# rezashkv/diffusion_pruning

Hardware: AMD Instinct MI355X
Metric: denoise-steps/s (SD-2.1 U-Net forward, 512x512, bs=4 per GPU, 50% channel mask) (higher is better)
Workload: dtype bf16; 1 GPU; BASELINE configs[1]: SD-2.1 UNet2DConditionModelGated.forward, 64x64 latents (512x512), bs=4/GPU, fixed 50% mask (gated semantics), seeded random-init weights, HIP graph replay; global_batch=4, parallelism=replicas x1 (no data-path collective)

## Files before the change

### diffusion_pruning_amd/_lib.py

```python
from __future__ import annotations

import ctypes
import os
from ctypes import POINTER, Structure, c_char_p, c_float, c_int, c_int32, c_int64, c_size_t, c_void_p

_HERE = os.path.dirname(os.path.abspath(__file__))
LIB_PATH = os.environ.get("APTP_LIB") or os.path.join(_HERE, "csrc", "libaptp_hip.so")

ACT_NONE, ACT_SILU, ACT_GEGLU, ACT_GELU = 0, 1, 2, 3
ACT_QUICK_GELU = 5
TILE_AUTO, TILE_128x128, TILE_128x160, TILE_64x128, TILE_64x160, TILE_128x64, TILE_64x64 = range(7)
(TILE_DMA_128x128, TILE_DMA_128x160, TILE_DMA_64x128, TILE_DMA_64x160, TILE_DMA_128x64, TILE_DMA_64x64) = range(7, 13)
(TILE_DMA3_128x128, TILE_DMA3_128x160, TILE_DMA3_64x128, TILE_DMA3_64x160, TILE_DMA3_128x64, TILE_DMA3_64x64) = range(13, 19)
TILE_DMA4_64x128, TILE_DMA4_64x64, TILE_DMA4_128x64 = 24, 25, 26
TILE_HALO_128x160, TILE_HALO_128x128 = 43, 44
(TILE_DMA6_64x64, TILE_DMA8S_64x64, TILE_DMA6_64x128, TILE_DMA6_128x64, TILE_KU2S4_64x64, TILE_KU2S6_64x64, TILE_KU2S4_64x128,
 TILE_KU2S6_64x128, TILE_KU2S4_128x64) = range(45, 54)
TILE_SK_256x160, TILE_SK_256x128 = 64, 65


class ConvGemmParams(Structure):
    _fields_ = [
        ("x", c_void_p), ("ldx", c_int64),
        ("B", c_int32), ("Hin", c_int32), ("Win", c_int32), ("Cin", c_int32),
# ... 26 lines not shown
        ("io_f32", c_int32),
        ("ustat_out", c_void_p), ("ustat_unit", c_int32), ("ustat_units", c_int32), ("ustat_nrep", c_int32),
        ("pad_end", c_int32),
    ]


class GroupNormColStats(Structure):
    _fields_ = [("stats", c_void_p), ("ld", c_int32), ("rows_per_block", c_int32), ("C", c_int32),
                ("ustats", c_void_p), ("unit", c_int32), ("units", c_int32), ("nrep", c_int32)]


class GroupNormParams(Structure):
    _fields_ = [
        ("x", c_void_p), ("ldx", c_int64),
        ("y", c_void_p), ("ldy", c_int64),
        ("B", c_int32), ("HW", c_int32), ("C", c_int32), ("groups", c_int32),
        ("gamma", c_void_p), ("beta", c_void_p),
        ("eps", c_float), ("silu", c_int32),
        ("workspace", c_void_p), ("variant", c_int32),
        ("counters", c_void_p),
        ("colstats", GroupNormColStats * 2),
        ("io_f32", c_int32),
    ]


class LayerNormParams(Structure):
    _fields_ = [
        ("x", c_void_p), ("ldx", c_int64),
        ("y", c_void_p), ("ldy", c_int64),
        ("rows", c_int32), ("C", c_int32),
        ("gamma", c_void_p), ("beta", c_void_p),
        ("eps", c_float),
        ("io_f32", c_int32),
    ]


class AttentionParams(Structure):
    _fields_ = [
        ("q", c_void_p), ("q_stride_b", c_int64), ("q_stride_l", c_int64),
        ("k", c_void_p), ("k_stride_b", c_int64), ("k_stride_l", c_int64),
        ("v", c_void_p), ("v_stride_b", c_int64), ("v_stride_l", c_int64),
        ("o", c_void_p), ("o_stride_b", c_int64), ("o_stride_l", c_int64),
        ("B", c_int32), ("heads", c_int32), ("Lq", c_int32), ("Lk", c_int32),
        ("scale", c_float),
        ("lse", c_void_p),
        ("variant", c_int32),
        ("io_f32", c_int32),
    ]


class GateBwdParams(Structure):
    _fields_ = [
        ("dy", c_void_p), ("lddy", c_int64), ("y0", c_void_p), ("ldy0", c_int64), ("dx", c_void_p), ("lddx", c_int64),
        ("B", c_int32), ("HW", c_int32), ("C", c_int32), ("groups", c_int32),
        ("gate", c_void_p), ("gate_B", c_int32),
        ("dgate_partial", c_void_p),
        ("dgate", c_void_p),
    ]


class GegluParams(Structure):
    _fields_ = [
        ("hg", c_void_p), ("ldhg", c_int64), ("out", c_void_p), ("ldout", c_int64),
        ("dout", c_void_p), ("lddout", c_int64), ("dhg", c_void_p), ("lddhg", c_int64),
        ("B", c_int32), ("HW", c_int32), ("C", c_int32), ("groups", c_int32),
        ("gate", c_void_p), ("gate_B", c_int32),
        ("dgate_partial", c_void_p),
        ("backward", c_int32),
        ("dgate", c_void_p),
    ]


class FfTailParams(Structure):
    _fields_ = [
        ("h", c_void_p), ("ldh", c_int64), ("x", c_void_p), ("ldx", c_int64), ("y", c_void_p), ("ldy", c_int64),
        ("w1", c_void_p), ("b1", c_void_p), ("cs1", c_void_p), ("n1", c_int32), ("ld1", c_int32),
        ("w2", c_void_p), ("b2", c_void_p), ("ld2", c_int32),
        ("w3", c_void_p), ("b3", c_void_p), ("ld3", c_int32),
        ("colstat", c_void_p), ("colstat_ld", c_int32),
        ("M", c_int32), ("C", c_int32),
        ("eps", c_float),
    ]


class WgradParams(Structure):
    _fields_ = [
        ("x", c_void_p), ("ldx", c_int64), ("dy", c_void_p), ("lddy", c_int64), ("dw", c_void_p),
        ("B", c_int32), ("H", c_int32), ("W", c_int32), ("C", c_int32), ("N", c_int32), ("KH", c_int32), ("KW", c_int32),
        ("split_m", c_int32), ("ld_dw", c_int32), ("db", c_void_p), ("slab_stride", c_int64), ("db_stride", c_int64),
        ("stride", c_int32), ("ups", c_int32),
    ]


class FoldRowsParams(Structure):
    _fields_ = [("partials", c_void_p), ("out", c_void_p), ("R", c_int32), ("n_rows", c_int32), ("C", c_int32), ("ld_out", c_int32),
                ("tail_out", c_void_p), ("tail_rows", c_int32), ("pair_split", c_int32), ("tail_n", c_int32)]


class PackDgradParams(Structure):
    _fields_ = [("src", c_void_p), ("dst", c_void_p), ("N", c_int32), ("C", c_int32), ("taps", c_int32), ("src_ld", c_int32),
                ("dst_ld", c_int32), ("dst_rows", c_int32)]


class DepthLerpParams(Structure):
    _fields_ = [
        ("x_in", c_void_p), ("ld_in", c_int64), ("x_out", c_void_p), ("ld_out", c_int64), ("y", c_void_p), ("ld_y", c_int64),
        ("dy", c_void_p), ("ld_dy", c_int64), ("d_in", c_void_p), ("ld_d_in", c_int64), ("d_out", c_void_p), ("ld_d_out", c_int64),
        ("B", c_int32), ("HW", c_int32), ("C", c_int32),
        ("d", c_void_p), ("d_B", c_int32),
        ("dd_partial", c_void_p),
        ("dd", c_void_p),
        ("backward", c_int32),
    ]


class AdamWItem(Structure):
    _fields_ = [("p", c_void_p), ("g", c_void_p), ("m", c_void_p), ("v", c_void_p), ("shadow", c_void_p), ("n", c_int64)]


class AdamWParams(Structure):
    _fields_ = [("items_dev", c_void_p), ("starts_dev", c_void_p), ("n_items", c_int32), ("total_blocks", c_int32),
                ("lr", c_float), ("beta1", c_float), ("beta2", c_float), ("eps", c_float), ("weight_decay", c_float),
                ("step_dev", c_void_p), ("gate_dev", c_void_p), ("grad_scale", c_float)]


class MseParams(Structure):
    _fields_ = [
        ("a", c_void_p), ("lda", c_int64), ("b", c_void_p), ("ldb", c_int64),
        ("rows", c_int64), ("C", c_int32), ("f32", c_int32),
        ("partial", c_void_p), ("out", c_void_p),
        ("g", c_void_p), ("da", c_void_p), ("ldda", c_int64),
        ("backward", c_int32),
    ]


class GroupNormBwdParams(Structure):
    _fields_ = [
        ("x", c_void_p), ("ldx", c_int64), ("dy", c_void_p), ("lddy", c_int64), ("dx", c_void_p), ("lddx", c_int64),
        ("B", c_int32), ("HW", c_int32), ("C", c_int32), ("groups", c_int32),
        ("gamma", c_void_p), ("beta", c_void_p),
        ("eps", c_float), ("silu", c_int32),
        ("fwd_stats", c_void_p),
        ("workspace", c_void_p),
        ("pgrad_partial", c_void_p),
        ("add", c_void_p), ("ldadd", c_int64),
    ]


class UnetPrologueParams(Structure):
    _fields_ = [
        ("sample", c_void_p), ("sample_bf16", c_int32), ("x", c_void_p),
        ("B", c_int32), ("C", c_int32), ("H", c_int32), ("W", c_int32), ("cin_pad", c_int32),
        ("timesteps", c_void_p), ("freqs", c_void_p), ("half", c_int32), ("t_emb", c_void_p),
    ]


class UnetEpilogueParams(Structure):
    _fields_ = [
        ("y", c_void_p), ("ldy", c_int64), ("out", c_void_p), ("out_bf16", c_int32),
        ("B", c_int32), ("C", c_int32), ("H", c_int32), ("W", c_int32),
    ]


class AttentionWideParams(Structure):
    _fields_ = [
        ("q", c_void_p), ("q_stride_b", c_int64), ("q_stride_l", c_int64),
        ("k", c_void_p), ("k_stride_b", c_int64), ("k_stride_l", c_int64),
        ("v", c_void_p), ("v_stride_b", c_int64), ("v_stride_l", c_int64),
        ("o", c_void_p), ("o_stride_b", c_int64), ("o_stride_l", c_int64),
        ("B", c_int32), ("Lq", c_int32), ("Lk", c_int32),
        ("scale", c_float),
        ("io_f32", c_int32),
    ]


class ImageOutParams(Structure):
    _fields_ = [
        ("y", c_void_p), ("ldy", c_int64), ("out", c_void_p), ("out_u8", c_int32),
        ("B", c_int32), ("H", c_int32), ("W", c_int32),
    ]


class ImageInParams(Structure):
    _fields_ = [
        ("x", c_void_p), ("x_bf16", c_int32), ("out", c_void_p), ("out_f32", c_int32),
        ("B", c_int32), ("C", c_int32), ("H", c_int32), ("W", c_int32),
    ]


class LatentDistParams(Structure):
    _fields_ = [
        ("y", c_void_p), ("ldy", c_int64), ("wq", c_void_p), ("bq", c_void_p), ("moments", c_void_p), ("eps", c_void_p),
        ("latents", c_void_p), ("latents_bf16", c_int32), ("scale", c_float),
        ("B", c_int32), ("H", c_int32), ("W", c_int32),
    ]


class AttentionCausalParams(Structure):
    _fields_ = [
        ("q", c_void_p), ("q_stride_b", c_int64), ("q_stride_l", c_int64),
        ("k", c_void_p), ("k_stride_b", c_int64), ("k_stride_l", c_int64),
        ("v", c_void_p), ("v_stride_b", c_int64), ("v_stride_l", c_int64),
        ("o", c_void_p), ("o_stride_b", c_int64), ("o_stride_l", c_int64),
        ("B", c_int32), ("heads", c_int32), ("L", c_int32),
        ("scale", c_float),
        ("io_f32", c_int32),
    ]


class TokenEmbedParams(Structure):
    _fields_ = [
        ("ids", c_void_p), ("tok", c_void_p), ("pos", c_void_p), ("out", c_void_p), ("ldo", c_int64),
        ("B", c_int32), ("L", c_int32), ("C", c_int32), ("vocab", c_int32), ("out_f32", c_int32), ("pos_rows", c_int32),
    ]


class AttentionBiasParams(Structure):
    _fields_ = [
        ("q", c_void_p), ("q_stride_b", c_int64), ("q_stride_l", c_int64),
        ("k", c_void_p), ("k_stride_b", c_int64), ("k_stride_l", c_int64),
        ("v", c_void_p), ("v_stride_b", c_int64), ("v_stride_l", c_int64),
        ("o", c_void_p), ("o_stride_b", c_int64), ("o_stride_l", c_int64),
        ("relbias", c_void_p), ("key_mask", c_void_p),
        ("B", c_int32), ("heads", c_int32), ("L", c_int32),
        ("scale", c_float),
        ("io_f32", c_int32),
    ]


class EmbedLnParams(Structure):
    _fields_ = [
        ("ids", c_void_p), ("word", c_void_p), ("pos", c_void_p), ("gamma", c_void_p), ("beta", c_void_p),
        ("out", c_void_p), ("ldo", c_int64),
        ("B", c_int32), ("L", c_int32), ("C", c_int32), ("vocab", c_int32), ("pos_rows", c_int32), ("pad_id", c_int32),
        ("out_f32", c_int32), ("eps", c_float),
    ]


class MaskedMeanParams(Structure):
    _fields_ = [
        ("x", c_void_p), ("x_stride_b", c_int64), ("x_stride_l", c_int64), ("mask", c_void_p), ("out", c_void_p),
        ("B", c_int32), ("L", c_int32), ("C", c_int32), ("x_f32", c_int32),
    ]


class ColsumParams(Structure):
    _fields_ = [("x", c_void_p), ("ldx", c_int64), ("rows", c_int32), ("C", c_int32), ("partial", c_void_p), ("batch", c_int32)]


class LayerNormPgradParams(Structure):
    _fields_ = [
        ("x", c_void_p), ("ldx", c_int64), ("dy", c_void_p), ("lddy", c_int64),
        ("rows", c_int32), ("C", c_int32), ("eps", c_float), ("partial", c_void_p),
    ]


class LayerNormBwdParams(Structure):
    _fields_ = [
        ("x", c_void_p), ("ldx", c_int64), ("dy", c_void_p), ("lddy", c_int64), ("dx", c_void_p), ("lddx", c_int64),
        ("rows", c_int32), ("C", c_int32),
        ("gamma", c_void_p),
        ("eps", c_float),
        ("add", c_void_p), ("ldadd", c_int64),
    ]


class AttentionBwdParams(Structure):
    _fields_ = [
        ("q", c_void_p), ("q_stride_b", c_int64), ("q_stride_l", c_int64),
        ("k", c_void_p), ("k_stride_b", c_int64), ("k_stride_l", c_int64),
        ("v", c_void_p), ("v_stride_b", c_int64), ("v_stride_l", c_int64),
        ("o", c_void_p), ("o_stride_b", c_int64), ("o_stride_l", c_int64),
        ("dout", c_void_p), ("dout_stride_b", c_int64), ("dout_stride_l", c_int64),
        ("dq", c_void_p), ("dq_stride_b", c_int64), ("dq_stride_l", c_int64),
        ("dk", c_void_p), ("dk_stride_b", c_int64), ("dk_stride_l", c_int64),
        ("dv", c_void_p), ("dv_stride_b", c_int64), ("dv_stride_l", c_int64),
        ("lse", c_void_p), ("delta", c_void_p),
        ("B", c_int32), ("heads", c_int32), ("Lq", c_int32), ("Lk", c_int32),
        ("scale", c_float), ("q_split", c_int32), ("workspace", c_void_p),
    ]


class ImagePatchesParams(Structure):
    _fields_ = [
        ("x", c_void_p), ("nchw", c_int32),
        ("B", c_int32), ("H", c_int32), ("W", c_int32),
        ("S", c_int32), ("P", c_int32),
        ("resize", c_int32),
        ("mean", c_float * 3), ("std", c_float * 3),
        ("out", c_void_p), ("ldo", c_int64),
        ("out_f32", c_int32),
    ]


class VitEmbedLnParams(Structure):
    _fields_ = [
        ("patches", c_void_p), ("ldp", c_int64),
        ("cls", c_void_p), ("pos", c_void_p), ("gamma", c_void_p), ("beta", c_void_p),
        ("out", c_void_p), ("ldo", c_int64),
        ("B", c_int32), ("T", c_int32), ("C", c_int32),
        ("out_f32", c_int32),
        ("eps", c_float),
    ]


class L2NormalizeParams(Structure):
    _fields_ = [("x", c_void_p), ("ldx", c_int64), ("out", c_void_p), ("ldo", c_int64), ("n", c_int32), ("D", c_int32)]


class MmdRbfParams(Structure):
    _fields_ = [
        ("x", c_void_p), ("ldx", c_int64),
        ("y", c_void_p), ("ldy", c_int64),
# ... 10 lines not shown
        ("B", c_int32), ("H", c_int32), ("W", c_int32),
        ("S", c_int32), ("P", c_int32),
        ("xbounds", c_void_p), ("xweights", c_void_p), ("xk", c_int32),
        ("ybounds", c_void_p), ("yweights", c_void_p), ("yk", c_int32),
        ("scratch", c_void_p),
        ("mean", c_float * 3), ("std", c_float * 3),
        ("out", c_void_p), ("ldo", c_int64),
        ("out_f32", c_int32),
    ]


EOS_ARGMAX, EOS_FIRST = 0, 1


class EosPoolLnParams(Structure):
    _fields_ = [
        ("ids", c_void_p),
        ("x", c_void_p), ("x_stride_b", c_int64), ("x_stride_l", c_int64),
        ("gamma", c_void_p), ("beta", c_void_p),
        ("out", c_void_p),
        ("out_act", c_void_p), ("ldo_act", c_int64),
        ("index_out", c_void_p),
        ("B", c_int32), ("L", c_int32), ("C", c_int32),
        ("eos_mode", c_int32), ("eos_token_id", c_int32),
        ("x_f32", c_int32), ("act_f32", c_int32),
        ("eps", c_float),
    ]


class PairedCosineParams(Structure):
    _fields_ = [
        ("a", c_void_p), ("lda", c_int64),
        ("b", c_void_p), ("ldb", c_int64),
        ("cos_out", c_void_p),
        ("sum_out", c_void_p),
        ("n", c_int32), ("D", c_int32),
        ("accumulate", c_int32),
    ]


TRAIN_NO_TABLE = -1


class TrainImageDesc(Structure):
    _fields_ = [
        ("src_off", c_int64),
        ("scratch_off", c_int64),
        ("xtab_off", c_int64), ("ytab_off", c_int64),
        ("H", c_int32), ("W", c_int32),
        ("H1", c_int32), ("W1", c_int32),
        ("top", c_int32), ("left", c_int32), ("flip", c_int32),
        ("xk", c_int32), ("yk", c_int32),
        ("row0", c_int32), ("nrows", c_int32),
        ("reserved", c_int32),
    ]


class TrainImagesParams(Structure):
    _fields_ = [
        ("images", c_void_p), ("images_bytes", c_int64),
        ("desc", c_void_p),
        ("desc_dev", c_void_p),
        ("tables", c_void_p), ("tables_count", c_int64),
        ("scratch", c_void_p), ("scratch_bytes", c_int64),
        ("out", c_void_p),
        ("B", c_int32), ("R", c_int32),
        ("out_f32", c_int32),
    ]


STEP_NOISE_BF16, STEP_NOISE_F32 = 0, 1
STEP_DDIM, STEP_PNDM, STEP_DPMPP = 0, 1, 2
STEP_EPSILON, STEP_V_PREDICTION = 0, 1


class GuidedStepParams(Structure):
    _fields_ = [
        ("noise", c_void_p),
        ("sample", c_void_p),
        ("out", c_void_p),
        ("coef", c_void_p),
        ("slot", c_void_p),
        ("w", c_void_p),
        ("flags", c_void_p),
        ("E", c_void_p),
        ("saved", c_void_p),
        ("n", c_int64),
        ("b", c_int32), ("noise_rows", c_int32),
        ("noise_dtype", c_int32), ("scheduler", c_int32), ("prediction", c_int32), ("do_cfg", c_int32),
        ("guidance_scale", c_float), ("guidance_rescale", c_float),
    ]


PHILOX_F32, PHILOX_BF16, PHILOX_RAW = 0, 1, 2


class PhiloxNormalParams(Structure):
    _fields_ = [
        ("out", c_void_p),
        ("base", c_void_p),
        ("seeds_dev", c_void_p),
        ("draw_dev", c_void_p),
        ("scale_dev", c_void_p),
        ("n", c_int64), ("offset", c_int64), ("draw", c_int64),
        ("b", c_int32), ("out_kind", c_int32),
        ("scale", c_float),
    ]


EXPORTS = [
    ("aptp_conv_gemm", c_int, [POINTER(ConvGemmParams), c_void_p]),
    ("aptp_conv_gemm_workspace_bytes", c_int64, [POINTER(ConvGemmParams)]),
    ("aptp_conv_gemm_suggest_split_k", c_int, [POINTER(ConvGemmParams)]),
    ("aptp_conv_gemm_rowstat_slots", c_int, [POINTER(ConvGemmParams)]),
    ("aptp_conv_gemm_tiles", c_int, [POINTER(ConvGemmParams)]),
    ("aptp_conv_gemm_colstat_rows", c_int, [POINTER(ConvGemmParams)]),
    ("aptp_groupnorm", c_int, [POINTER(GroupNormParams), c_void_p]),
    ("aptp_groupnorm_nchunk", c_int, [c_int]),
    ("aptp_rows_nchunk", c_int, [c_int]),
    ("aptp_groupnorm_workspace_bytes", c_int64, [POINTER(GroupNormParams)]),
    ("aptp_layernorm", c_int, [POINTER(LayerNormParams), c_void_p]),
    ("aptp_attention", c_int, [POINTER(AttentionParams), c_void_p]),
    ("aptp_gate_bwd", c_int, [POINTER(GateBwdParams), c_void_p]),
    ("aptp_geglu", c_int, [POINTER(GegluParams), c_void_p]),
    ("aptp_depth_lerp", c_int, [POINTER(DepthLerpParams), c_void_p]),
    ("aptp_ff_tail_supported", c_int, [c_int, c_int, c_int, c_int, c_int, c_int]),
    ("aptp_ff_tail", c_int, [POINTER(FfTailParams), c_void_p]),
    ("aptp_conv_wgrad_supported", c_int, [POINTER(WgradParams)]),
    ("aptp_conv_wgrad_suggest_split", c_int, [POINTER(WgradParams)]),
    ("aptp_conv_wgrad", c_int, [POINTER(WgradParams), c_void_p]),
    ("aptp_conv_wgrad_many_item_bytes", ctypes.c_int64, []),
    ("aptp_conv_wgrad_many_blocks", c_int, [POINTER(WgradParams)]),
    ("aptp_conv_wgrad_many_fill", c_int, [POINTER(WgradParams), c_void_p, ctypes.c_int32]),
    ("aptp_conv_wgrad_many", c_int, [c_void_p, c_void_p, ctypes.c_int32, ctypes.c_int32, ctypes.c_int32, c_void_p]),
    ("aptp_fold_rows", c_int, [POINTER(FoldRowsParams), c_void_p]),
    ("aptp_pack_dgrad", c_int, [POINTER(PackDgradParams), c_void_p]),
    ("aptp_fold_rows_blocks", c_int, [POINTER(FoldRowsParams)]),
    ("aptp_fold_rows_many", c_int, [c_void_p, c_void_p, c_int32, c_int32, c_void_p]),
    ("aptp_pack_dgrad_blocks", c_int, [POINTER(PackDgradParams)]),
    ("aptp_pack_dgrad_many", c_int, [c_void_p, c_void_p, c_int32, c_int32, c_void_p]),
    ("aptp_adamw_blocks", c_int, [c_int64]),
    ("aptp_adamw_many", c_int, [POINTER(AdamWParams), c_void_p]),
    ("aptp_mse_nblocks", c_int, [c_int64, c_int32]),
    ("aptp_mse", c_int, [POINTER(MseParams), c_void_p]),
    ("aptp_groupnorm_bwd", c_int, [POINTER(GroupNormBwdParams), c_void_p]),
    ("aptp_layernorm_bwd", c_int, [POINTER(LayerNormBwdParams), c_void_p]),
    ("aptp_attention_bwd", c_int, [POINTER(AttentionBwdParams), c_void_p]),
    ("aptp_attention_bwd_q_split", c_int, [POINTER(AttentionBwdParams)]),
    ("aptp_attention_bwd_workspace_bytes", c_size_t, [POINTER(AttentionBwdParams), c_int32]),
    ("aptp_colsum", c_int, [POINTER(ColsumParams), c_void_p]),
    ("aptp_layernorm_pgrad", c_int, [POINTER(LayerNormPgradParams), c_void_p]),
    ("aptp_unet_prologue", c_int, [POINTER(UnetPrologueParams), c_void_p]),
    ("aptp_unet_epilogue", c_int, [POINTER(UnetEpilogueParams), c_void_p]),
    ("aptp_attention_wide", c_int, [POINTER(AttentionWideParams), c_void_p]),
    ("aptp_image_out", c_int, [POINTER(ImageOutParams), c_void_p]),
    ("aptp_image_in", c_int, [POINTER(ImageInParams), c_void_p]),
    ("aptp_latent_dist", c_int, [POINTER(LatentDistParams), c_void_p]),
    ("aptp_attention_causal", c_int, [POINTER(AttentionCausalParams), c_void_p]),
    ("aptp_token_embed", c_int, [POINTER(TokenEmbedParams), c_void_p]),
    ("aptp_attention_bias", c_int, [POINTER(AttentionBiasParams), c_void_p]),
    ("aptp_embed_ln", c_int, [POINTER(EmbedLnParams), c_void_p]),
    ("aptp_masked_mean", c_int, [POINTER(MaskedMeanParams), c_void_p]),
    ("aptp_image_patches", c_int, [POINTER(ImagePatchesParams), c_void_p]),
    ("aptp_vit_embed_ln", c_int, [POINTER(VitEmbedLnParams), c_void_p]),
    ("aptp_l2_normalize", c_int, [POINTER(L2NormalizeParams), c_void_p]),
    ("aptp_mmd_rbf_workspace_bytes", c_int64, [c_int32, c_int32]),
    ("aptp_mmd_rbf", c_int, [POINTER(MmdRbfParams), c_void_p]),
    ("aptp_image_patches_pil_size", c_int, [c_int32, c_int32, c_int32, POINTER(c_int32), POINTER(c_int32), POINTER(c_int32),
                                            POINTER(c_int32)]),
    ("aptp_image_patches_pil", c_int, [POINTER(ImagePatchesPilParams), c_void_p]),
    ("aptp_eos_pool_ln", c_int, [POINTER(EosPoolLnParams), c_void_p]),
    ("aptp_paired_cosine", c_int, [POINTER(PairedCosineParams), c_void_p]),
    ("aptp_train_images", c_int, [POINTER(TrainImagesParams), c_void_p]),
    ("aptp_guided_step", c_int, [POINTER(GuidedStepParams), c_void_p]),
    ("aptp_philox_normal", c_int, [POINTER(PhiloxNormalParams), c_void_p]),
    ("aptp_last_error", c_char_p, []),
    ("aptp_version", c_int, []),
]

_lib = None


class AptpError(RuntimeError):
    pass


def load():
    global _lib
    if _lib is not None:
        return _lib
    import torch
    if not os.path.exists(LIB_PATH):
        raise AptpError(
            f"{LIB_PATH} not found: the HIP extension is the only compute path of diffusion_pruning_amd. "
            "Build it with `make -C diffusion_pruning_amd/csrc` (hipcc, --offload-arch=gfx950).")
    lib = ctypes.CDLL(LIB_PATH)
    for name, res, args in EXPORTS:
        fn = getattr(lib, name)
        fn.restype = res
        fn.argtypes = args
    _lib = lib
    return lib


def check(rc: int, what: str):
    if rc != 0:
        msg = load().aptp_last_error()
        raise AptpError(f"{what} failed (rc={rc}): {msg.decode() if msg else ''}")
```

### diffusion_pruning_amd/csrc/conv_gemm.hip

```cpp
#include "conv_gemm_core.h"

using namespace aptp_cg;

namespace {

template <typename T> struct Elem;
template <> struct Elem<__bf16> { static constexpr int EPC = 8, KS = 64; };
template <> struct Elem<float> { static constexpr int EPC = 4, KS = 32; };

template <int BM, int BN, int WM, int WN, typename T = __bf16>
__global__ __launch_bounds__(256) void conv_gemm_kernel(const KParams p) {
  static_assert(WM * WN == 4, "4 waves per workgroup");
  constexpr int EPC = Elem<T>::EPC, KS = Elem<T>::KS, ES = (int)sizeof(T);
  constexpr bool F32 = sizeof(T) == 4;
  constexpr int WTM = BM / WM, WTN = BN / WN;
  constexpr int MF = WTM / 16, NF = WTN / 16;
  constexpr int A_PASS = BM / 32, B_PASS = BN / 32;
  static_assert(BM % 32 == 0 && BN % 32 == 0 && WTM % 16 == 0 && WTN % 16 == 0, "tile shape");

  __shared__ __attribute__((aligned(16))) T smem[2 * (BM + BN) * KS];
  T* As = smem;
  T* Bs = smem + 2 * BM * KS;

  const int tid = threadIdx.x, lane = tid & 63, wave = tid >> 6;
// ... 957 lines not shown
  k.x2 = (const __bf16*)p->x2; k.ldx2 = p->ldx2; k.Cin2 = p->x2 ? p->Cin2 : 0; k.ncc2 = p->x2 ? p->cin2_pad / ks : 0; k.x2_bytes = 0;
  if (p->x2) {
    APTP_CHECK(p->Cin2 > 0 && p->Cin2 % 8 == 0 && p->cin2_pad % BK == 0 && p->cin2_pad >= p->Cin2 && p->cin2_pad < p->Cin2 + BK,
               "conv_gemm: x2 needs Cin2 (%d) a positive multiple of 8 and cin2_pad (%d) == ceil(Cin2/64)*64", p->Cin2, p->cin2_pad);
    APTP_CHECK(p->ldx2 % 8 == 0 && p->ldx2 >= p->Cin2 && ((uintptr_t)p->x2 % 16) == 0, "conv_gemm: x2 row stride / alignment");
    APTP_CHECK(p->stride == 1 && p->ups == 0 && p->Hout == p->Hin && p->Wout == p->Win,
               "conv_gemm: x2 (second operand read at the output pixel) needs a stride-1, same-size convolution");
    const int64_t x2b = (((int64_t)p->B * p->Hout * p->Wout - 1) * p->ldx2 + p->Cin2) * es;
    APTP_CHECK(x2b < (1ll << 31), "conv_gemm: x2 larger than 2 GiB");
    k.x2_bytes = (int)x2b;
  }
  k.w = (const __bf16*)p->w; k.N = p->N; k.ncc = p->cin_pad / ks; k.nK = p->KH * p->KW * k.ncc + k.ncc2;
  k.Ktot = (int64_t)k.nK * ks;
  k.bias = p->bias; k.rowbias = p->rowbias; k.ld_rowbias = p->ld_rowbias;
  k.colgate = p->colgate; k.gate_group = p->gate_group; k.gate_B = p->gate_B;
  k.act = p->act; k.corr = p->corr; k.corr_B = p->corr_B;
  k.residual = (const __bf16*)p->residual; k.ldres = p->ldres;
  k.depth = p->depth; k.depth_B = p->depth_B; k.depth_in = (const __bf16*)p->depth_in; k.lddin = p->lddin;
  k.y = p->y; k.ldy = p->ldy; k.out_f32 = p->out_f32;
  k.split_k = p->split_k < k.nK ? p->split_k : k.nK;
  k.ws = (float*)p->workspace;
  k.M = (int)M64; k.HW = p->Hout * p->Wout; k.Nout = nout;
  k.ws_ld = p->N;
  APTP_CHECK(p->order >= 0 && p->order <= 3, "conv_gemm: order %d", p->order);
  if (p->order == 0) {
    const int64_t w_bytes = (int64_t)p->N * k.Ktot * 2;
    const int64_t a_bytes = (int64_t)p->B * p->Hin * p->Win * p->Cin * 2;
    k.order = w_bytes > a_bytes ? 1 : 2;
  } else {
    k.order = p->order - 1;
  }
  k.rstat_out = p->rowstat_out; k.rstat_slots = p->rowstat_slots;
  k.ln_stats = p->ln_stats; k.ln_slots = p->ln_slots; k.ln_colsum = p->ln_colsum; k.ln_eps = p->ln_eps;
  k.ln_invC = p->ln_C > 0 ? 1.0f / (float)p->ln_C : 0.f;
  APTP_CHECK(!p->rowstat_out || (!geglu && (!p->out_f32 || f32) && ((uintptr_t)p->rowstat_out % 16) == 0),
             "conv_gemm: rowstat_out needs a bf16, non-GEGLU output and an 8-byte aligned buffer");
  APTP_CHECK(!p->ln_stats || (p->ln_colsum && p->ln_slots > 0 && p->ln_C > 0 && p->KH == 1 && p->KW == 1 &&
                              p->ln_slots % 2 == 0 && ((uintptr_t)p->ln_stats % 16) == 0 && ((uintptr_t)p->ln_colsum % 16) == 0),
             "conv_gemm: folded LayerNorm needs ln_colsum [N], ln_slots > 0, ln_C > 0 and a 1x1 filter");
  k.counters = p->tile_counters;
  k.pf_ptr = ((uintptr_t)p->prefetch & 3) ? nullptr : (const char*)p->prefetch;
  k.pf_bytes = k.pf_ptr ? (p->prefetch_bytes < (1ll << 36) ? p->prefetch_bytes : (1ll << 36)) : 0;
  k.cstat_out = p->colstat_out; k.cstat_ld = p->colstat_ld;
  k.ustat_out = (long long*)p->ustat_out; k.ustat_unit = p->ustat_unit; k.ustat_units = p->ustat_units; k.ustat_nrep = p->ustat_nrep;
  APTP_CHECK(!p->ustat_out || (p->colstat_out && p->ustat_unit > 0 && p->ustat_units * p->ustat_unit >= nout && p->ustat_nrep >= 1 &&
                               (p->ustat_nrep & (p->ustat_nrep - 1)) == 0 && ((uintptr_t)p->ustat_out % 8) == 0),
             "conv_gemm: ustat_out goes with colstat_out; ustat_unit > 0, ustat_units >= ceil(N_out / unit), ustat_nrep a power of two");
  k.epi16 = !p->out_f32 && p->ldy % 8 == 0 && ((uintptr_t)p->y % 16) == 0 && nout % 8 == 0 &&
            (!p->residual || (p->ldres % 8 == 0 && ((uintptr_t)p->residual % 16) == 0)) &&
            (!p->depth || (p->lddin % 8 == 0 && ((uintptr_t)p->depth_in % 16) == 0));
  if (p->epilogue == 1) k.epi16 = 0;
  const int64_t xb = (((int64_t)p->B * p->Hin * p->Win - 1) * p->ldx + p->Cin) * es;
  const int64_t wb = (int64_t)p->N * k.Ktot * es;
  APTP_CHECK(xb < (1ll << 31) && wb < (1ll << 31), "conv_gemm: operand larger than 2 GiB");
  k.x_bytes = (int)xb; k.w_bytes = (int)wb;
  return APTP_OK;
}

template <int BM, int BN>
void launch_tile(const KParams& k, hipStream_t s) {
  const int tiles = ((k.M + BM - 1) / BM) * ((k.N + BN - 1) / BN);
  dim3 grid(tiles * k.split_k, 1, 1);
  if (k.io_f32) hipLaunchKernelGGL((conv_gemm_kernel<BM, BN, 2, 2, float>), grid, dim3(256), 0, s, k);
  else hipLaunchKernelGGL((conv_gemm_kernel<BM, BN, 2, 2>), grid, dim3(256), 0, s, k);
}

template <int BM, int BN, int STAGES>
void launch_tile_dma(const KParams& k, hipStream_t s) {
  const int tiles = ((k.M + BM - 1) / BM) * ((k.N + BN - 1) / BN);
  dim3 grid(tiles * k.split_k, 1, 1);
  hipLaunchKernelGGL((conv_gemm_dma_kernel<BM, BN, 2, 2, STAGES>), grid, dim3(256), 0, s, k);
}

template <int BM, int BN, int WM, int WN, int STAGES = 2>
void launch_tile_dma8(const KParams& k, hipStream_t s) {
  const int tiles = ((k.M + BM - 1) / BM) * ((k.N + BN - 1) / BN);
  dim3 grid(tiles * k.split_k, 1, 1);
  hipLaunchKernelGGL((conv_gemm_dma_kernel<BM, BN, WM, WN, STAGES>), grid, dim3(512), 0, s, k);
}

template <int BM, int BN, int WM, int WN, int STAGES>
void launch_tile_ku2(const KParams& k, hipStream_t s) {
  const int tiles = ((k.M + BM - 1) / BM) * ((k.N + BN - 1) / BN);
  dim3 grid(tiles * k.split_k, 1, 1);
  hipLaunchKernelGGL((conv_gemm_dma_kernel<BM, BN, WM, WN, STAGES, false, 2>), grid, dim3(WM * WN * 64), 0, s, k);
}

template <int BM, int BN, int STAGES>
void launch_tile_ks2(const KParams& k, hipStream_t s) {
  const int tiles = ((k.M + BM - 1) / BM) * ((k.N + BN - 1) / BN);
  dim3 grid(tiles * k.split_k, 1, 1);
  hipLaunchKernelGGL((conv_gemm_dma_kernel<BM, BN, 2, 2, STAGES, false, 1, 2>), grid, dim3(512), 0, s, k);
}

template <int BM, int BN, int WM, int WN, int STAGES>
void launch_tile_pp(const KParams& k, hipStream_t s) {
  const int tiles = ((k.M + BM - 1) / BM) * ((k.N + BN - 1) / BN);
  dim3 grid(tiles * k.split_k, 1, 1);
  hipLaunchKernelGGL((conv_gemm_dma_kernel<BM, BN, WM, WN, STAGES, true>), grid, dim3(512), 0, s, k);
}

}

extern "C" int64_t aptp_conv_gemm_workspace_bytes(const AptpConvGemmParams* p) {
  if (!p || p->split_k <= 1) return 0;
  const int64_t M = (int64_t)p->B * p->Hout * p->Wout;
  const int t = pick_tile(p, (int)M);
  if (is_sk_tile(t))
    return (int64_t)aptp_sk_cus() * 2 * kTiles[t].bm * kTiles[t].bn * (int64_t)sizeof(float);
  int64_t mp = M, np = p->N;
  if (t > 0 && t < kNumTiles) {
    mp = (M + kTiles[t].bm - 1) / kTiles[t].bm * kTiles[t].bm;
    np = ((int64_t)p->N + kTiles[t].bn - 1) / kTiles[t].bn * kTiles[t].bn;
  }
  return (int64_t)p->split_k * mp * np * (int64_t)sizeof(float);
}

extern "C" int aptp_conv_gemm_tiles(const AptpConvGemmParams* p) {
  if (!p) return 0;
  const int64_t M = (int64_t)p->B * p->Hout * p->Wout;
  const int t = pick_tile(p, (int)M);
  if (t <= 0 || t >= kNumTiles) return 0;
  return (int)(((M + kTiles[t].bm - 1) / kTiles[t].bm) * ((p->N + kTiles[t].bn - 1) / kTiles[t].bn));
}

extern "C" int aptp_conv_gemm_colstat_rows(const AptpConvGemmParams* p) {
  if (!p) return 0;
  const int t = pick_tile(p, p->B * p->Hout * p->Wout);
  if (t <= 0 || t >= kNumTiles) return 0;
  return kTiles[t].bm / (kTiles[t].nw / kTiles[t].wn);
}

extern "C" int aptp_conv_gemm_rowstat_slots(const AptpConvGemmParams* p) {
  if (!p) return 0;
  const int t = pick_tile(p, p->B * p->Hout * p->Wout);
  if (t <= 0 || t >= kNumTiles) return 0;
  return ((p->N + kTiles[t].bn - 1) / kTiles[t].bn) * kTiles[t].wn;
}

extern "C" int aptp_conv_gemm_suggest_split_k(const AptpConvGemmParams* p) {
  if (!p) return 1;
  const int M = p->B * p->Hout * p->Wout;
  const int t = pick_tile(p, M);
  const int64_t blocks = (int64_t)((M + kTiles[t].bm - 1) / kTiles[t].bm) * ((p->N + kTiles[t].bn - 1) / kTiles[t].bn);
  const int nK = p->KH * p->KW * (p->cin_pad / BK);
  if (blocks >= 256) return 1;
  int s = (int)((512 + blocks - 1) / blocks);
  const int max_s = nK / 8 > 0 ? nK / 8 : 1;
  if (s > max_s) s = max_s;
  if (s > 32) s = 32;
  return s < 1 ? 1 : s;
}

extern "C" int aptp_conv_gemm(const AptpConvGemmParams* p, aptp_stream_t stream) {
  KParams k;
  const int rc = fill_kparams(p, k);
  if (rc != APTP_OK) return rc;
  if (k.split_k > 1) APTP_CHECK(k.ws != nullptr && ((uintptr_t)k.ws % 16) == 0, "conv_gemm: split_k > 1 needs a 16B-aligned workspace");
  if (k.split_k == 1) k.counters = nullptr;
  k.gn_gamma = p->gn_gamma; k.gn_beta = p->gn_beta; k.gn_groups = p->gn_groups; k.gn_C = p->gn_C; k.gn_silu = p->gn_silu; k.gn_eps = p->gn_eps;
  if (k.gn_gamma) {
    APTP_CHECK(k.gn_beta && k.split_k > 1 && !k.counters && !k.out_f32 && k.act == APTP_ACT_NONE && !k.colgate && !k.corr && !k.residual && !k.depth
               && !k.rstat_out && !k.cstat_out && !k.ln_stats, "conv_gemm: gn_gamma needs a plain bf16 convolution split along K with a reduce launch");
    APTP_CHECK(k.gn_groups > 0 && k.gn_C > 0 && k.gn_C <= k.N && k.gn_C % k.gn_groups == 0 && k.gn_C % 8 == 0 && (k.gn_C / k.gn_groups) % 4 == 0
               && (int64_t)k.HW * (k.gn_C / k.gn_groups) <= 4LL * GN_RED_QPT * GN_RED_NT && k.ldy % 4 == 0,
               "conv_gemm: gn_gamma geometry (C=%d groups=%d HW=%d)", k.gn_C, k.gn_groups, k.HW);
  }
  hipStream_t s = (hipStream_t)stream;
  int t = pick_tile(p, k.M);
  if (t < 0 || t >= kNumTiles) { aptp_set_error("conv_gemm: unknown tile %d", t); return APTP_EINVAL; }
  if (k.io_f32 && t >= APTP_TILE_DMA_128x128) {
    aptp_set_error("conv_gemm: io_f32 (fp32 parity path) runs on the register-staged tiles 1..6 only (got tile %d)", t);
    return APTP_EINVAL;
  }
  if (t >= APTP_TILE_DMA_128x128 && !is_sk_tile(t) && (p->cin_pad * 2 > 8064 || (p->x2 && p->cin2_pad * 2 > 8064))) {
    aptp_set_error("conv_gemm: LDS-DMA tiles need Cin <= 4032 (got cin_pad %d)", p->cin_pad);
    return APTP_EINVAL;
  }
  if (k.rstat_out) {
    const int slots = ((k.N + kTiles[t].bn - 1) / kTiles[t].bn) * kTiles[t].wn;
    if ((k.split_k != 1 && !k.counters) || k.rstat_slots != slots) {
      aptp_set_error("conv_gemm: rowstat_out needs split_k == 1 (or the in-kernel reduction) and rowstat_slots == aptp_conv_gemm_rowstat_slots() (%d), got split_k %d, slots %d",
                     slots, k.split_k, k.rstat_slots);
      return APTP_EINVAL;
    }
  }
  if (k.cstat_out) {
    const int wtm = kTiles[t].bm / (kTiles[t].nw / kTiles[t].wn), wtn = kTiles[t].bn / kTiles[t].wn;
    if (!k.epi16 || k.act == APTP_ACT_GEGLU || (k.split_k != 1 && !k.counters) || k.HW % wtm != 0 || wtn < 32 ||
        k.cstat_ld < k.Nout || ((uintptr_t)k.cstat_out % 8) != 0) {
      aptp_set_error("conv_gemm: colstat_out needs the coalesced bf16 epilogue, no GEGLU, split_k == 1 (or the in-kernel reduction), "
                     "Hout*Wout %% %d == 0 (aptp_conv_gemm_colstat_rows) and colstat_ld >= N", wtm);
      return APTP_EINVAL;
    }
    const int wl = k.act == APTP_ACT_GEGLU ? wtn / 2 : wtn;
    if (k.ustat_out && (wl % k.ustat_unit == 0 ? wl / k.ustat_unit : (wl - 1) / k.ustat_unit + 2) > 64) {
      aptp_set_error("conv_gemm: ustat_unit %d too small for the %d columns of a wave of tile %d (at most 64 units per wave)", k.ustat_unit, wl, t);
      return APTP_EINVAL;
    }
  }
  if (k.act == APTP_ACT_GEGLU && (kTiles[t].bn == 160)) {
    aptp_set_error("conv_gemm: GEGLU cannot use a 160-wide tile");
    return APTP_EINVAL;
  }
  {
    const int tiles_m = (k.M + kTiles[t].bm - 1) / kTiles[t].bm, tiles_n = (k.N + kTiles[t].bn - 1) / kTiles[t].bn;
    APTP_CHECK((int64_t)tiles_m * tiles_n * k.split_k < (1ll << 31) && (int64_t)k.nK * (k.split_k + 1) < (1ll << 31), "conv_gemm: grid too large");
    k.fd_hw = make_fastdiv(k.HW); k.fd_wout = make_fastdiv(k.Wout);
    k.fd_tm = make_fastdiv(tiles_m); k.fd_tn = make_fastdiv(tiles_n); k.fd_sk = make_fastdiv(k.split_k);
    k.fd_perm = make_fastdiv(tiles_n * k.split_k); k.fd_tmn = make_fastdiv(tiles_m * tiles_n);
  }
  static const bool lin_on = !(getenv("APTP_LIN") && getenv("APTP_LIN")[0] == '0');
  if (lin_on && p->epilogue != 2 && p->pad_end == 0 && aptp_lin_eligible(k, t)) {
    const int rc2 = aptp_launch_lin(k, t, s);
    if (rc2 != APTP_OK) return rc2;
    APTP_LAUNCH_CHECK();
    return APTP_OK;
  }
  static const bool lean_on = !(getenv("APTP_CONV_LEAN") && getenv("APTP_CONV_LEAN")[0] == '0');
  if (lean_on && p->epilogue == 0 && p->pad_end == 0 && aptp_conv_lean_eligible(k, t)) {
    const int rc2 = aptp_launch_conv_lean(k, t, s);
    if (rc2 != APTP_OK) return rc2;
  } else
  switch (t) {
    case APTP_TILE_128x128: launch_tile<128, 128>(k, s); break;
    case APTP_TILE_128x160: launch_tile<128, 160>(k, s); break;
    case APTP_TILE_64x128: launch_tile<64, 128>(k, s); break;
    case APTP_TILE_64x160: launch_tile<64, 160>(k, s); break;
    case APTP_TILE_128x64: launch_tile<128, 64>(k, s); break;
    case APTP_TILE_64x64: launch_tile<64, 64>(k, s); break;
    case APTP_TILE_DMA_128x128: launch_tile_dma<128, 128, 2>(k, s); break;
    case APTP_TILE_DMA_128x160: launch_tile_dma<128, 160, 2>(k, s); break;
    case APTP_TILE_DMA_64x128: launch_tile_dma<64, 128, 2>(k, s); break;
    case APTP_TILE_DMA_64x160: launch_tile_dma<64, 160, 2>(k, s); break;
    case APTP_TILE_DMA_128x64: launch_tile_dma<128, 64, 2>(k, s); break;
    case APTP_TILE_DMA_64x64: launch_tile_dma<64, 64, 2>(k, s); break;
    case APTP_TILE_DMA3_128x128: launch_tile_dma<128, 128, 3>(k, s); break;
    case APTP_TILE_DMA3_128x160: launch_tile_dma<128, 160, 3>(k, s); break;
    case APTP_TILE_DMA3_64x128: launch_tile_dma<64, 128, 3>(k, s); break;
    case APTP_TILE_DMA3_64x160: launch_tile_dma<64, 160, 3>(k, s); break;
    case APTP_TILE_DMA3_128x64: launch_tile_dma<128, 64, 3>(k, s); break;
    case APTP_TILE_DMA3_64x64: launch_tile_dma<64, 64, 3>(k, s); break;
    case APTP_TILE_DMA8_128x160: launch_tile_dma8<128, 160, 4, 2>(k, s); break;
    case APTP_TILE_DMA8_256x160: launch_tile_dma8<256, 160, 4, 2>(k, s); break;
    case APTP_TILE_DMA8_128x128: launch_tile_dma8<128, 128, 2, 4>(k, s); break;
    case APTP_TILE_DMA8_256x128: launch_tile_dma8<256, 128, 4, 2>(k, s); break;
    case APTP_TILE_DMA4_64x160: launch_tile_dma<64, 160, 4>(k, s); break;
    case APTP_TILE_DMA4_64x128: launch_tile_dma<64, 128, 4>(k, s); break;
    case APTP_TILE_DMA4_64x64: launch_tile_dma<64, 64, 4>(k, s); break;
    case APTP_TILE_DMA4_128x64: launch_tile_dma<128, 64, 4>(k, s); break;
    case APTP_TILE_DMA4_128x128: launch_tile_dma<128, 128, 4>(k, s); break;
    case APTP_TILE_DMA8R3_128x160: launch_tile_dma8<128, 160, 4, 2, 3>(k, s); break;
    case APTP_TILE_DMA8R4_128x160: launch_tile_dma8<128, 160, 4, 2, 4>(k, s); break;
    case APTP_TILE_DMA8R3_128x128: launch_tile_dma8<128, 128, 2, 4, 3>(k, s); break;
    case APTP_TILE_DMA8R4_128x128: launch_tile_dma8<128, 128, 2, 4, 4>(k, s); break;
    case APTP_TILE_DMA8R3_256x128: launch_tile_dma8<256, 128, 4, 2, 3>(k, s); break;
    case APTP_TILE_PP3_128x160: launch_tile_pp<128, 160, 4, 2, 3>(k, s); break;
    case APTP_TILE_PP4_128x160: launch_tile_pp<128, 160, 4, 2, 4>(k, s); break;
    case APTP_TILE_PP3_128x128: launch_tile_pp<128, 128, 2, 4, 3>(k, s); break;
    case APTP_TILE_PP4_128x128: launch_tile_pp<128, 128, 2, 4, 4>(k, s); break;
    case APTP_TILE_PP4_64x160: launch_tile_pp<64, 160, 4, 2, 4>(k, s); break;
    case APTP_TILE_PP4_64x128: launch_tile_pp<64, 128, 2, 4, 4>(k, s); break;
    case APTP_TILE_PP5_64x160: launch_tile_pp<64, 160, 4, 2, 5>(k, s); break;
    case APTP_TILE_PP4_128x64: launch_tile_pp<128, 64, 4, 2, 4>(k, s); break;
    case APTP_TILE_PP3_256x128: launch_tile_pp<256, 128, 4, 2, 3>(k, s); break;
    case APTP_TILE_PP3_128x256: launch_tile_pp<128, 256, 2, 4, 3>(k, s); break;
    case APTP_TILE_DMA6_64x64: launch_tile_dma<64, 64, 6>(k, s); break;
    case APTP_TILE_DMA8S_64x64: launch_tile_dma<64, 64, 8>(k, s); break;
    case APTP_TILE_DMA6_64x128: launch_tile_dma<64, 128, 6>(k, s); break;
    case APTP_TILE_DMA6_128x64: launch_tile_dma<128, 64, 6>(k, s); break;
    case APTP_TILE_KU2S4_64x64: launch_tile_ku2<64, 64, 2, 2, 4>(k, s); break;
    case APTP_TILE_KU2S6_64x64: launch_tile_ku2<64, 64, 2, 2, 6>(k, s); break;
    case APTP_TILE_KU2S4_64x128: launch_tile_ku2<64, 128, 2, 2, 4>(k, s); break;
    case APTP_TILE_KU2S6_64x128: launch_tile_ku2<64, 128, 2, 2, 6>(k, s); break;
    case APTP_TILE_KU2S4_128x64: launch_tile_ku2<128, 64, 2, 2, 4>(k, s); break;
    case APTP_TILE_KU2S4_128x128: launch_tile_ku2<128, 128, 2, 2, 4>(k, s); break;
    case APTP_TILE_KU2S4_64x160: launch_tile_ku2<64, 160, 2, 2, 4>(k, s); break;
    case APTP_TILE_KU2S4_128x160: launch_tile_ku2<128, 160, 4, 2, 4>(k, s); break;
    case APTP_TILE_KU2S4_128x128W8: launch_tile_ku2<128, 128, 2, 4, 4>(k, s); break;
    case APTP_TILE_KS2S3_64x64: launch_tile_ks2<64, 64, 3>(k, s); break;
    case APTP_TILE_KS2S4_64x64: launch_tile_ks2<64, 64, 4>(k, s); break;
    case APTP_TILE_KS2S3_64x128: launch_tile_ks2<64, 128, 3>(k, s); break;
    case APTP_TILE_KS2S4_64x128: launch_tile_ks2<64, 128, 4>(k, s); break;
    case APTP_TILE_KS2S3_128x64: launch_tile_ks2<128, 64, 3>(k, s); break;
    case APTP_TILE_KS2S3_128x128: launch_tile_ks2<128, 128, 3>(k, s); break;
    case APTP_TILE_SK_256x160: case APTP_TILE_SK_256x128: case APTP_TILE_SK_128x256:
    case APTP_TILE_SKL_256x160: case APTP_TILE_SKL_256x128: case APTP_TILE_SKL_128x256:
    case APTP_TILE_SK_128x160: case APTP_TILE_SKL_128x160: case APTP_TILE_SK_128x128: case APTP_TILE_SKL_128x128: {
      if (k.split_k > 1 && !k.counters) { aptp_set_error("conv_gemm: the stream-K tiles combine in-kernel: split_k > 1 needs tile_counters"); return APTP_EINVAL; }
      const int rc2 = aptp_launch_sk(k, t, s);
      if (rc2 != APTP_OK) return rc2;
      break;
    }
    case APTP_TILE_HALO_128x160:
    case APTP_TILE_HALO_128x128: {
      const int W = p->Wout;
      if (!(p->KH == 3 && p->KW == 3 && p->stride == 1 && p->pad == 1 && p->pad_end == 0 && p->ups == 0 && !p->x2 && W > 0 && 128 % W == 0 &&
            (p->Hout * W) % 128 == 0 && (128 / W + 2) * (W + 2) <= 264)) {
        aptp_set_error("conv_gemm: the halo tiles need a 3x3 / stride-1 / pad-1 convolution without x2 whose width divides 128 (16, 32 or 64)");
        return APTP_EINVAL;
      }
      const int tiles = ((k.M + 127) / 128) * ((k.N + kTiles[t].bn - 1) / kTiles[t].bn);
      if (t == APTP_TILE_HALO_128x160) hipLaunchKernelGGL((conv3x3_halo_kernel<160, 4>), dim3(tiles * k.split_k), dim3(512), 0, s, k);
      else hipLaunchKernelGGL((conv3x3_halo_kernel<128, 4>), dim3(tiles * k.split_k), dim3(512), 0, s, k);
      break;
    }
    default: aptp_set_error("conv_gemm: unknown tile %d", t); return APTP_EINVAL;
  }
  APTP_LAUNCH_CHECK();
  if (k.split_k > 1 && !k.counters) {
    if (k.gn_gamma) {
      hipLaunchKernelGGL(splitk_reduce_gn_kernel, dim3(k.gn_groups, k.B), dim3(GN_RED_NT), 0, s, k);
    } else {
      const int quads = (k.act == APTP_ACT_GEGLU) ? k.N / 8 : k.N / 4;
      const int64_t total = (int64_t)k.M * quads;
      hipLaunchKernelGGL(splitk_reduce_kernel, dim3((unsigned)((total + 255) / 256)), dim3(256), 0, s, k);
    }
    APTP_LAUNCH_CHECK();
  }
  return APTP_OK;
}
```

### diffusion_pruning_amd/csrc/unet_io.hip

```cpp
#include "aptp_common.h"

namespace {

struct IoK {
  const void* sample; int sample_bf16; void* x; int B, C, HW, cpad;
  const float* t; const float* freqs; int half; void* temb;
  int pix_blocks;
};

__global__ __launch_bounds__(256) void unet_prologue_kernel(const IoK p) {
  const int tid = threadIdx.x;
  if ((int)blockIdx.x < p.pix_blocks) {
    const int64_t pix = (int64_t)blockIdx.x * 256 + tid;
    if (pix >= (int64_t)p.B * p.HW) return;
    const int b = (int)(pix / p.HW), r = (int)(pix - (int64_t)b * p.HW);
    __bf16* dst = reinterpret_cast<__bf16*>(p.x) + pix * p.cpad;
    for (int c0 = 0; c0 < p.cpad; c0 += 8) {
      float f[8];
#pragma unroll
      for (int e = 0; e < 8; ++e) {
        const int c = c0 + e;
        float v = 0.f;
        if (c < p.C) {
          const int64_t i = ((int64_t)b * p.C + c) * p.HW + r;
          v = p.sample_bf16 ? (float)reinterpret_cast<const __bf16*>(p.sample)[i] : reinterpret_cast<const float*>(p.sample)[i];
        }
        f[e] = v;
      }
      *reinterpret_cast<uint4*>(dst + c0) = pack_bf16x8(f);
    }
    return;
  }
  const int i = ((int)blockIdx.x - p.pix_blocks) * 256 + tid;
  if (i >= p.B * p.half) return;
  const int b = i / p.half, k = i - b * p.half;
  const float a = p.t[b] * p.freqs[k];
  __bf16* e = reinterpret_cast<__bf16*>(p.temb) + (int64_t)b * 2 * p.half;
  e[k] = (__bf16)cosf(a);
  e[p.half + k] = (__bf16)sinf(a);
}

struct OutK { const float* y; int64_t ld; void* out; int out_bf16; int B, C, HW; };

__global__ __launch_bounds__(256) void unet_epilogue_kernel(const OutK p) {
  const int64_t i = (int64_t)blockIdx.x * 256 + threadIdx.x;
  if (i >= (int64_t)p.B * p.C * p.HW) return;
  const int r = (int)(i % p.HW);
  const int64_t bc = i / p.HW;
  const int c = (int)(bc % p.C), b = (int)(bc / p.C);
  const float v = p.y[((int64_t)b * p.HW + r) * p.ld + c];
  if (p.out_bf16) reinterpret_cast<__bf16*>(p.out)[i] = (__bf16)v;
  else reinterpret_cast<float*>(p.out)[i] = v;
}

struct ImgK { const float* y; int64_t ld; void* out; int out_u8; int B, HW; };

__global__ __launch_bounds__(256) void image_out_kernel(const ImgK p) {
  const int64_t i = (int64_t)blockIdx.x * 256 + threadIdx.x;
  if (i >= (int64_t)p.B * 3 * p.HW) return;
  int64_t pix;
  int c;
  if (p.out_u8) {
    pix = i / 3;
    c = (int)(i - pix * 3);
  } else {
    const int r = (int)(i % p.HW);
    const int64_t bc = i / p.HW;
    c = (int)(bc % 3);
    pix = (bc / 3) * p.HW + r;
  }
  const float y = p.y[pix * p.ld + c];
  const float v = fminf(fmaxf(__fadd_rn(__fmul_rn(y, 0.5f), 0.5f), 0.f), 1.f);
  if (p.out_u8) reinterpret_cast<uint8_t*>(p.out)[i] = (uint8_t)rintf(__fmul_rn(v, 255.f));
  else reinterpret_cast<float*>(p.out)[i] = v;
}

struct ImgInK { const void* x; int x_bf16; void* out; int out_f32; int B, H, W; };

__global__ __launch_bounds__(256) void image_in_kernel(const ImgInK p) {
  const int64_t pix = (int64_t)blockIdx.x * 256 + threadIdx.x;
  const int64_t HW = (int64_t)p.H * p.W;
  if (pix >= (int64_t)p.B * HW) return;
  const int b = (int)(pix / HW), r = (int)(pix - (int64_t)b * HW);
  const int oy = r / p.W, ox = r - oy * p.W;
  float v[32];
#pragma unroll
  for (int e = 27; e < 32; ++e) v[e] = 0.f;
#pragma unroll
  for (int ky = 0; ky < 3; ++ky) {
#pragma unroll
    for (int kx = 0; kx < 3; ++kx) {
      const int iy = oy + ky - 1, ix = ox + kx - 1;
      const bool ok = (unsigned)iy < (unsigned)p.H && (unsigned)ix < (unsigned)p.W;
#pragma unroll
      for (int c = 0; c < 3; ++c) {
        float f = 0.f;
        if (ok) {
          const int64_t i = ((int64_t)b * 3 + c) * HW + (int64_t)iy * p.W + ix;
          f = p.x_bf16 ? (float)reinterpret_cast<const __bf16*>(p.x)[i] : reinterpret_cast<const float*>(p.x)[i];
        }
        v[(ky * 3 + kx) * 3 + c] = f;
      }
    }
  }
  if (p.out_f32) {
    float4* dst = reinterpret_cast<float4*>(reinterpret_cast<float*>(p.out) + pix * 32);
#pragma unroll
    for (int q = 0; q < 8; ++q) dst[q] = make_float4(v[4 * q], v[4 * q + 1], v[4 * q + 2], v[4 * q + 3]);
  } else {
    uint4* dst = reinterpret_cast<uint4*>(reinterpret_cast<__bf16*>(p.out) + pix * 32);
#pragma unroll
    for (int q = 0; q < 4; ++q) dst[q] = pack_bf16x8(v + 8 * q);
  }
}

struct LatK { const float* y; int64_t ld; const float* wq; const float* bq; float* mom; const float* eps; void* lat; int lat_bf16;
              float scale; int B, HW; };

__global__ __launch_bounds__(256) void latent_dist_kernel(const LatK p) {
  const int64_t pix = (int64_t)blockIdx.x * 256 + threadIdx.x;
  if (pix >= (int64_t)p.B * p.HW) return;
  const int b = (int)(pix / p.HW), r = (int)(pix - (int64_t)b * p.HW);
  const float4* src = reinterpret_cast<const float4*>(p.y + pix * p.ld);
  const float4 y0 = src[0], y1 = src[1];
  const float y[8] = {y0.x, y0.y, y0.z, y0.w, y1.x, y1.y, y1.z, y1.w};
  float m[8];
#pragma unroll
  for (int o = 0; o < 8; ++o) {
    float acc = __fmul_rn(p.wq[o * 8], y[0]);
#pragma unroll
    for (int i = 1; i < 8; ++i) acc = __fadd_rn(acc, __fmul_rn(p.wq[o * 8 + i], y[i]));
    m[o] = __fadd_rn(acc, p.bq[o]);
  }
  const int64_t base8 = (int64_t)b * 8 * p.HW + r;
  if (p.mom) {
#pragma unroll
    for (int o = 0; o < 8; ++o) p.mom[base8 + (int64_t)o * p.HW] = m[o];
  }
  if (p.eps) {
    const int64_t base4 = (int64_t)b * 4 * p.HW + r;
#pragma unroll
    for (int c = 0; c < 4; ++c) {
      const float lv = fminf(fmaxf(m[4 + c], -30.f), 20.f);
      const float sd = expf(__fmul_rn(0.5f, lv));
      const float z = __fmul_rn(p.scale, __fadd_rn(m[c], __fmul_rn(sd, p.eps[base4 + (int64_t)c * p.HW])));
      if (p.lat_bf16) reinterpret_cast<__bf16*>(p.lat)[base4 + (int64_t)c * p.HW] = (__bf16)z;
      else reinterpret_cast<float*>(p.lat)[base4 + (int64_t)c * p.HW] = z;
    }
  }
}

struct TokK { const int64_t* ids; const float* tok; const float* pos; void* out; int64_t ldo; int L, C, vocab, out_f32; };

__global__ __launch_bounds__(128) void token_embed_kernel(const TokK p) {
  const int64_t row = blockIdx.x;
  const int l = (int)(row % p.L);
  const int64_t id = p.ids[row];
  const bool ok = id >= 0 && id < p.vocab;
  const float* tr = p.tok + (ok ? id : 0) * (int64_t)p.C;
  const float* pr = p.pos + (int64_t)l * p.C;
  for (int c = 8 * threadIdx.x; c < p.C; c += 8 * 128) {
    float v[8];
    if (ok) {
      const float4 t0 = *reinterpret_cast<const float4*>(tr + c), t1 = *reinterpret_cast<const float4*>(tr + c + 4);
      const float4 q0 = *reinterpret_cast<const float4*>(pr + c), q1 = *reinterpret_cast<const float4*>(pr + c + 4);
      v[0] = __fadd_rn(t0.x, q0.x); v[1] = __fadd_rn(t0.y, q0.y); v[2] = __fadd_rn(t0.z, q0.z); v[3] = __fadd_rn(t0.w, q0.w);
      v[4] = __fadd_rn(t1.x, q1.x); v[5] = __fadd_rn(t1.y, q1.y); v[6] = __fadd_rn(t1.z, q1.z); v[7] = __fadd_rn(t1.w, q1.w);
    } else {
#pragma unroll
      for (int e = 0; e < 8; ++e) v[e] = __builtin_nanf("");
    }
    if (p.out_f32) {
      float4* dst = reinterpret_cast<float4*>(reinterpret_cast<float*>(p.out) + row * p.ldo + c);
      dst[0] = make_float4(v[0], v[1], v[2], v[3]);
      dst[1] = make_float4(v[4], v[5], v[6], v[7]);
    } else {
      *reinterpret_cast<uint4*>(reinterpret_cast<__bf16*>(p.out) + row * p.ldo + c) = pack_bf16x8(v);
    }
  }
}

}

extern "C" int aptp_image_in(const AptpImageInParams* p, aptp_stream_t stream) {
  APTP_CHECK(p && p->x && p->out, "image_in: null pointer");
  APTP_CHECK(p->C == 3, "image_in: pixel_values must have 3 channels (got %d)", p->C);
  APTP_CHECK(p->B > 0 && p->H > 0 && p->W > 0, "image_in: bad extents");
  APTP_CHECK(((uintptr_t)p->x % (p->x_bf16 ? 2 : 4)) == 0 && ((uintptr_t)p->out % 16) == 0, "image_in: pointer alignment");
  const int64_t pix = (int64_t)p->B * p->H * p->W;
  APTP_CHECK((pix + 255) / 256 < (1ll << 31), "image_in: too many pixels");
  ImgInK k;
  k.x = p->x; k.x_bf16 = p->x_bf16 ? 1 : 0; k.out = p->out; k.out_f32 = p->out_f32 ? 1 : 0; k.B = p->B; k.H = p->H; k.W = p->W;
  hipLaunchKernelGGL(image_in_kernel, dim3((unsigned)((pix + 255) / 256)), dim3(256), 0, (hipStream_t)stream, k);
  APTP_LAUNCH_CHECK();
  return APTP_OK;
}

extern "C" int aptp_latent_dist(const AptpLatentDistParams* p, aptp_stream_t stream) {
  APTP_CHECK(p && p->y && p->wq && p->bq, "latent_dist: null pointer");
  APTP_CHECK(p->moments || p->eps, "latent_dist: nothing to write (moments and eps both NULL)");
  APTP_CHECK(!p->eps || p->latents, "latent_dist: eps needs latents");
  APTP_CHECK(p->B > 0 && p->H > 0 && p->W > 0 && p->ldy >= 8 && p->ldy % 4 == 0, "latent_dist: bad extents (ldy >= 8, a multiple of 4)");
  APTP_CHECK(((uintptr_t)p->y % 16) == 0 && ((uintptr_t)p->wq % 4) == 0 && ((uintptr_t)p->bq % 4) == 0 &&
             ((uintptr_t)p->moments % 4) == 0 && ((uintptr_t)p->eps % 4) == 0 && ((uintptr_t)p->latents % (p->latents_bf16 ? 2 : 4)) == 0,
             "latent_dist: pointer alignment");
  APTP_CHECK(p->scale == p->scale, "latent_dist: scale is NaN");
  const int64_t pix = (int64_t)p->B * p->H * p->W;
  APTP_CHECK((int64_t)p->H * p->W < (1ll << 31) && (pix + 255) / 256 < (1ll << 31), "latent_dist: too many pixels");
  LatK k;
  k.y = p->y; k.ld = p->ldy; k.wq = p->wq; k.bq = p->bq; k.mom = p->moments; k.eps = p->eps; k.lat = p->latents;
  k.lat_bf16 = p->latents_bf16 ? 1 : 0; k.scale = p->scale; k.B = p->B; k.HW = p->H * p->W;
  hipLaunchKernelGGL(latent_dist_kernel, dim3((unsigned)((pix + 255) / 256)), dim3(256), 0, (hipStream_t)stream, k);
  APTP_LAUNCH_CHECK();
  return APTP_OK;
}

extern "C" int aptp_image_out(const AptpImageOutParams* p, aptp_stream_t stream) {
  APTP_CHECK(p && p->y && p->out, "image_out: null pointer");
  APTP_CHECK(p->B > 0 && p->H > 0 && p->W > 0 && p->ldy >= 3, "image_out: bad extents (ldy >= 3)");
  APTP_CHECK(((uintptr_t)p->y % 4) == 0 && (p->out_u8 || ((uintptr_t)p->out % 4) == 0), "image_out: pointer alignment");
  APTP_CHECK((int64_t)p->H * p->W < (1ll << 31), "image_out: H * W too large");
  ImgK k;
  k.y = p->y; k.ld = p->ldy; k.out = p->out; k.out_u8 = p->out_u8 ? 1 : 0; k.B = p->B; k.HW = p->H * p->W;
  const int64_t n = (int64_t)k.B * 3 * k.HW;
  APTP_CHECK((n + 255) / 256 < (1ll << 31), "image_out: too many elements");
  hipLaunchKernelGGL(image_out_kernel, dim3((unsigned)((n + 255) / 256)), dim3(256), 0, (hipStream_t)stream, k);
  APTP_LAUNCH_CHECK();
  return APTP_OK;
}

extern "C" int aptp_unet_prologue(const AptpUnetPrologueParams* p, aptp_stream_t stream) {
  APTP_CHECK(p && p->sample && p->x && p->timesteps && p->freqs && p->t_emb, "unet_prologue: null pointer");
  APTP_CHECK(p->B > 0 && p->C > 0 && p->H > 0 && p->W > 0 && p->cin_pad >= p->C && p->cin_pad % 8 == 0 && p->half > 0,
             "unet_prologue: bad extents (cin_pad must be a multiple of 8 and >= C)");
  APTP_CHECK(((uintptr_t)p->x % 16) == 0, "unet_prologue: x alignment");
  IoK k;
  k.sample = p->sample; k.sample_bf16 = p->sample_bf16; k.x = p->x; k.B = p->B; k.C = p->C; k.HW = p->H * p->W; k.cpad = p->cin_pad;
  k.t = p->timesteps; k.freqs = p->freqs; k.half = p->half; k.temb = p->t_emb;
  const int64_t pix = (int64_t)p->B * k.HW;
  k.pix_blocks = (int)((pix + 255) / 256);
  const int tblocks = (p->B * p->half + 255) / 256;
  hipLaunchKernelGGL(unet_prologue_kernel, dim3(k.pix_blocks + tblocks), dim3(256), 0, (hipStream_t)stream, k);
  APTP_LAUNCH_CHECK();
  return APTP_OK;
}

extern "C" int aptp_unet_epilogue(const AptpUnetEpilogueParams* p, aptp_stream_t stream) {
  APTP_CHECK(p && p->y && p->out, "unet_epilogue: null pointer");
  APTP_CHECK(p->B > 0 && p->C > 0 && p->H > 0 && p->W > 0 && p->ldy >= p->C, "unet_epilogue: bad extents");
  OutK k;
  k.y = p->y; k.ld = p->ldy; k.out = p->out; k.out_bf16 = p->out_bf16; k.B = p->B; k.C = p->C; k.HW = p->H * p->W;
  const int64_t n = (int64_t)k.B * k.C * k.HW;
  hipLaunchKernelGGL(unet_epilogue_kernel, dim3((unsigned)((n + 255) / 256)), dim3(256), 0, (hipStream_t)stream, k);
  APTP_LAUNCH_CHECK();
  return APTP_OK;
}

extern "C" int aptp_token_embed(const AptpTokenEmbedParams* p, aptp_stream_t stream) {
  APTP_CHECK(p && p->ids && p->tok && p->pos && p->out, "token_embed: null pointer");
  APTP_CHECK(p->B > 0 && p->L > 0 && p->vocab > 0 && p->C > 0 && p->C % 8 == 0, "token_embed: bad extents (C must be a multiple of 8)");
  APTP_CHECK(p->L <= p->pos_rows, "token_embed: %d tokens but only %d position rows", p->L, p->pos_rows);
  APTP_CHECK(p->ldo >= p->C && p->ldo % 8 == 0, "token_embed: ldo (%lld) must be >= C and a multiple of 8", (long long)p->ldo);
  APTP_CHECK((int64_t)p->B * p->L < (1ll << 31), "token_embed: B * L too large");
  APTP_CHECK(((uintptr_t)p->ids % 8) == 0 && ((uintptr_t)p->tok % 16) == 0 && ((uintptr_t)p->pos % 16) == 0 && ((uintptr_t)p->out % 16) == 0,
             "token_embed: pointer alignment");
  TokK k;
  k.ids = p->ids; k.tok = p->tok; k.pos = p->pos; k.out = p->out; k.ldo = p->ldo;
  k.L = p->L; k.C = p->C; k.vocab = p->vocab; k.out_f32 = p->out_f32;
  hipLaunchKernelGGL(token_embed_kernel, dim3((unsigned)(p->B * p->L)), dim3(128), 0, (hipStream_t)stream, k);
  APTP_LAUNCH_CHECK();
  return APTP_OK;
}
```

### diffusion_pruning_amd/ops.py

```python
from __future__ import annotations

import ctypes
import os
import threading
from dataclasses import dataclass
from typing import Optional

import torch

from . import _lib
from ._lib import ImageInParams, LatentDistParams, UnetEpilogueParams, UnetPrologueParams
from ._lib import ACT_GELU, AttentionCausalParams, TokenEmbedParams
from ._lib import AttentionBiasParams, EmbedLnParams, MaskedMeanParams
from ._lib import ACT_QUICK_GELU, ImagePatchesParams, L2NormalizeParams, MmdRbfParams, VitEmbedLnParams
from ._lib import EOS_ARGMAX, EOS_FIRST, EosPoolLnParams, ImagePatchesPilParams, PairedCosineParams
from ._lib import GuidedStepParams, PhiloxNormalParams
from ._lib import (ACT_GEGLU, ACT_NONE, ACT_SILU, AttentionBwdParams, AttentionParams, ConvGemmParams, DepthLerpParams, GateBwdParams, WgradParams, FfTailParams, FoldRowsParams, PackDgradParams, MseParams,
                   GegluParams, GroupNormBwdParams, GroupNormParams, LayerNormBwdParams, LayerNormParams,
                   ColsumParams, LayerNormPgradParams, AttentionWideParams, ImageOutParams)
from .launch_policy import (BK, SK_AUTO, SK_TILE_FIRST, TUNING, _HALO_TILES, choose_launch, key_of, parse_key,
                            set_entry, set_tuning, splitk_in_kernel, tuning_key, tuning_lookup)

ACT_DTYPE = torch.bfloat16

# ... 94 lines not shown

        def padrows(t):
            if t.shape[0] == n_p:
                return t
            return torch.cat([t, t.new_zeros((n_p - t.shape[0],) + tuple(t.shape[1:]))], 0)
        wh, wg = padrows(wh), padrows(wg)
        w = torch.stack([wh.reshape(n_p // 16, 16, *wh.shape[1:]), wg.reshape(n_p // 16, 16, *wg.shape[1:])], 1)
        w = w.reshape(2 * n_p, *wh.shape[1:])
        if bias is not None:
            bh, bg = padrows(bh), padrows(bg)
            bias = torch.stack([bh.reshape(n_p // 16, 16), bg.reshape(n_p // 16, 16)], 1).reshape(2 * n_p)
    else:
        if out_idx is not None:
            out_idx = out_idx.to(device)
            w = w[out_idx]
            if bias is not None:
                bias = bias[out_idx]
        if in_idx is not None:
            w = w[:, in_idx.to(device)]
        n_live = w.shape[0]
        n_p = round_up(n_live, n_pad_to)
        if n_p != n_live:
            w = torch.cat([w, w.new_zeros((n_p - n_live,) + tuple(w.shape[1:]))], 0)
            if bias is not None:
                bias = torch.cat([bias, bias.new_zeros(n_p - n_live)], 0)
    N, Cin, KH, KW = w.shape
    cin_live = round_up(Cin, cin_pad_to)
    cin_pad = round_up(cin_live, BK)
    packed = torch.zeros(N, KH * KW, cin_pad, dtype=ACT_DTYPE, device=device)
    packed[:, :, :Cin] = w.permute(0, 2, 3, 1).reshape(N, KH * KW, Cin).to(ACT_DTYPE)
    colsum = packed.float().sum(dim=(1, 2)).contiguous() if ln_gamma is not None else None
    return PackedWeight(packed.contiguous(), None if bias is None else bias.contiguous(), N, cin_live, KH, KW, geglu, colsum)


def pack_weight_cat(pw: PackedWeight, w2: torch.Tensor, bias2: Optional[torch.Tensor] = None, *,
                    in_idx: Optional[torch.Tensor] = None) -> PackedWeight:
    assert not pw.geglu and pw.ln_colsum is None and pw.Cin2 == 0
    dev = pw.w.device
    w2 = w2.to(device=dev, dtype=torch.float32).reshape(w2.shape[0], -1)
    if in_idx is not None:
        w2 = w2[:, in_idx.to(dev)]
    n_live, c2 = w2.shape
    assert n_live <= pw.N
    c2_live = round_up(c2, 8)
    c2_pad = round_up(c2_live, BK)
    ext = torch.zeros(pw.N, c2_pad, dtype=ACT_DTYPE, device=dev)
    ext[:n_live, :c2] = w2.to(ACT_DTYPE)
    flat = torch.cat([pw.w.reshape(pw.N, -1), ext], 1).reshape(pw.N, 1, -1).contiguous()
    bias = pw.bias
    if bias2 is not None:
        b2 = torch.zeros(pw.N, dtype=torch.float32, device=dev)
        b2[:n_live] = bias2.to(device=dev, dtype=torch.float32)
        bias = b2 if bias is None else bias + b2
    return PackedWeight(flat, bias, pw.N, pw.Cin, pw.KH, pw.KW, False, None, c2_live, c2_pad, pw.cin_pad)


_ws_cache = {}
_ws_capture_keep = []

LAUNCH_LOG = None
GN_LAUNCH_LOG = None
ATTN_LAUNCH_LOG = None

SPLITK_IN_KERNEL = True
_counters = {}
_N_COUNTERS = 1 << 16


_N_SLABS = int(os.environ.get("APTP_N_SLABS", "16"))
_counters_lock = threading.Lock()


class scratch_domain:

    def __init__(self, name):
        self.name = name

    def __enter__(self):
        self.prev = getattr(_tls, "domain", None)
        _tls.domain = self.name
        return self

    def __exit__(self, *exc):
        _tls.domain = self.prev
        return False


def _domain():
    return getattr(_tls, "domain", None)


def _tile_counters(device):
    key = device.index if device.index is not None else torch.cuda.current_device()
    pool = _counters.get(key)
    if pool is None:
        if torch.cuda.is_current_stream_capturing():
            return None
        with _counters_lock:
            pool = _counters.get(key)
            if pool is None:
                pool = {"buf": torch.zeros(_N_SLABS, _N_COUNTERS, dtype=torch.int32, device=device), "slab": {}}
                _counters[key] = pool
    sid = (torch.cuda.current_stream().cuda_stream, _domain())
    i = pool["slab"].get(sid)
    if i is None:
        with _counters_lock:
            i = pool["slab"].get(sid)
            if i is None:
                if len(pool["slab"]) >= _N_SLABS:
                    return None
                i = pool["slab"][sid] = len(pool["slab"])
    return pool["buf"][i]


GN_DEFAULT_VARIANT = 0
GN_STATS_ONE_LAUNCH = True

ATTN_VARIANT = int(os.environ.get("APTP_ATTN_VARIANT", "0"))

GN_FUSED_FINALIZE = False

EPILOGUE = 0


def _workspace(nbytes: int, device) -> torch.Tensor:
    key = (device.index if device.index is not None else torch.cuda.current_device(), torch.cuda.is_current_stream_capturing(),
           torch.cuda.current_stream().cuda_stream, _domain())
    buf = _ws_cache.get(key)
    if buf is None or buf.numel() < nbytes:
        size = max(nbytes, 1 << 20)
        if key[1] and buf is not None:
            size = max(size, buf.numel() + buf.numel() // 2)
        buf = torch.empty(size, dtype=torch.uint8, device=device)
        if key[1]:
            _ws_capture_keep.append(buf)
        _ws_cache[key] = buf
    return buf


COLSTATS = True
COLSTATS_MIN_HW = 1024


def _root(t: torch.Tensor) -> torch.Tensor:
    return t._base if t._base is not None else t


USTAT = os.environ.get("APTP_USTAT", "1") != "0"
USTAT_NREP = int(os.environ.get("APTP_USTAT_NREP", "8"))
_USTAT_WORDS = 1 << 17
_ustat_arenas = {}


def ustat_begin(device, unit: int):
    if not USTAT or unit <= 0 or torch.device(device).type != "cuda":
        _tls.ustat = None
        return
    capturing = torch.cuda.is_current_stream_capturing()
    key = (torch.device(device).index, torch.cuda.current_stream().cuda_stream, _domain(), capturing)
    ent = _ustat_arenas.get(key)
    if ent is None:
        ent = _ustat_arenas[key] = {"buf": torch.zeros(_USTAT_WORDS, dtype=torch.int64, device=device), "used": 0}
        if capturing:
            _ws_capture_keep.append(ent["buf"])
            ent["used"] = _USTAT_WORDS
    elif ent["used"]:
        ent["buf"][:ent["used"]].zero_()
    _tls.ustat = {"buf": ent["buf"], "off": 0, "unit": int(unit), "ent": ent}


def ustat_end():
    st = getattr(_tls, "ustat", None)
    if st is not None and not st.get("closed"):
        st["closed"] = True
        st["ent"]["used"] = max(st["ent"]["used"], st["off"])


def _ustat_alloc(B: int, nout: int):
    st = getattr(_tls, "ustat", None)
    if st is None or st.get("closed"):
        return None
    unit = st["unit"]
    units = (nout + unit - 1) // unit
    nrep = USTAT_NREP
    while nrep > 1 and nrep * B > 4 * USTAT_NREP:
        nrep //= 2
    n = nrep * B * units * 2
    if st["off"] + n > st["buf"].numel():
        return None
    u = st["buf"][st["off"]:st["off"] + n]
    st["off"] += n
    return u, unit, units, nrep


def _colstats_drop(out: torch.Tensor):
    d = getattr(_root(out), "_aptp_colstats", None)
    if d:
        d.pop(out.storage_offset(), None)


def _colstats_put(out: torch.Tensor, stats: torch.Tensor, rows_per_block: int, ustat=None):
    root = _root(out)
    d = getattr(root, "_aptp_colstats", None)
    if d is None:
        d = {}
        root._aptp_colstats = d
    d[out.storage_offset()] = (stats, rows_per_block, out.shape[3], (out.shape[0], out.shape[1] * out.shape[2]), _ld(out), ustat)


def _colstats_get(x: torch.Tensor, C: int):
    d = getattr(_root(x), "_aptp_colstats", None)
    if not d:
        return None
    segs, off, left, pad = [], x.storage_offset(), x.shape[3], x.shape[3] - C
    while left > 0 and len(segs) < 2:
        rec = d.get(off)
        if rec is None or rec[3] != (x.shape[0], x.shape[1] * x.shape[2]) or rec[4] != _ld(x) or rec[2] > left:
            return None
        segs.append([rec[0], rec[1], rec[2], rec[5] if len(rec) > 5 else None])
        off += rec[2]
        left -= rec[2]
    if left != 0 or segs[-1][2] <= pad:
        return None
    segs[-1][2] -= pad
    return segs


class _PrefetchPlan:

    def __init__(self):
        self.seq = []
        self.i = 0

    def begin(self):
        self.i = 0

    def step(self, w):
        i, self.i = self.i, self.i + 1
        if i < len(self.seq) and self.seq[i] is w:
            nxt = self.seq[i + 1] if i + 1 < len(self.seq) else None
        else:
            del self.seq[i:]
            self.seq.append(w)
            nxt = None
        if nxt is not None and not (PREFETCH_MIN_BYTES <= nxt.numel() * nxt.element_size() <= PREFETCH_MAX_BYTES):
            return None
        return nxt


_tls = threading.local()


def set_prefetch_plan(plan: Optional[_PrefetchPlan]):
    _tls.prefetch_plan = plan
    if plan is not None:
        plan.begin()


def _current_prefetch_plan() -> Optional[_PrefetchPlan]:
    return getattr(_tls, "prefetch_plan", None)


PREFETCH_WEIGHTS = os.environ.get("APTP_PREFETCH", "1") == "1"
PREFETCH_MIN_BYTES = int(os.environ.get("APTP_PREFETCH_MIN", "0"))
PREFETCH_MAX_BYTES = int(os.environ.get("APTP_PREFETCH_MAX", str(12 << 20)))


def conv_gemm(x: torch.Tensor, pw: PackedWeight, *, stride: int = 1, pad: Optional[int] = None, ups: int = 0,
              out: Optional[torch.Tensor] = None, rowbias: Optional[torch.Tensor] = None,
              colgate: Optional[torch.Tensor] = None, gate_group: int = 0, act: int = ACT_NONE,
              corr: Optional[torch.Tensor] = None, residual: Optional[torch.Tensor] = None,
              depth: Optional[torch.Tensor] = None, depth_in: Optional[torch.Tensor] = None,
              out_f32: bool = False, split_k: Optional[int] = None, tile: int = 0, order: int = 0,
              rowstats: bool = False, ln=None, colstats: bool = False, x2: Optional[torch.Tensor] = None,
              prefetch=None, gn=None, pad_end: int = 0):
    if pad_end < 0 or (pad_end and (ups or corr is not None or x2 is not None)):
        raise ValueError("conv_gemm: pad_end must be >= 0 and does not go with ups, corr or x2")
    lib = _lib.load()
    if gn is not None and (colgate is not None or act != ACT_NONE or pw.geglu or corr is not None or residual is not None
                           or depth is not None or out_f32 or rowstats or ln is not None or out is not None):
        raise ValueError("conv_gemm: gn= goes with a plain bf16 convolution (bias / rowbias only)")
    _check_act(x, "conv_gemm x")
    B, Hin, Win, Cx = x.shape
    if Cx != pw.Cin:
        raise ValueError(f"conv_gemm: x has {Cx} channels, packed weight expects {pw.Cin}")
    if pad is None:
        pad = pw.KH // 2
    sh = 1 if ups else 0
    HinE, WinE = Hin << sh, Win << sh
    Hout = (HinE + 2 * pad + pad_end - pw.KH) // stride + 1
    Wout = (WinE + 2 * pad + pad_end - pw.KW) // stride + 1
    if pw.geglu:
        act = ACT_GEGLU
    nout = pw.N // 2 if act == ACT_GEGLU else pw.N
    f32 = x.dtype == torch.float32
    gn_f32 = None
    if f32:
        if pw.w.dtype != torch.float32:
            raise ValueError("conv_gemm: fp32 activations need weights packed under ops.ACT_DTYPE = torch.float32")
        out_f32, colstats, prefetch, gn_f32, gn = True, False, False, gn, None
        if tile not in (0, 1, 2, 3, 4, 5, 6):
            raise ValueError("conv_gemm: the fp32 parity path runs on the register-staged tiles 1..6")
    if out is None:
        out = torch.empty(B, Hout, Wout, nout, dtype=torch.float32 if out_f32 else torch.bfloat16, device=x.device)
    else:
        _colstats_drop(out)
        if tuple(out.shape) != (B, Hout, Wout, nout) or out.stride(3) != 1:
            raise ValueError(f"conv_gemm: out shape {tuple(out.shape)} != {(B, Hout, Wout, nout)}")
        if out.dtype != (torch.float32 if out_f32 else torch.bfloat16):
            raise ValueError("conv_gemm: out dtype mismatch")
    p = ConvGemmParams()
    p.x, p.ldx = x.data_ptr(), _ld(x)
    p.B, p.Hin, p.Win, p.Cin, p.Hout, p.Wout = B, Hin, Win, Cx, Hout, Wout
    p.KH, p.KW, p.stride, p.pad, p.ups = pw.KH, pw.KW, stride, pad, ups
    p.pad_end = pad_end
    p.w, p.N, p.cin_pad = pw.w.data_ptr(), pw.N, pw.cin_pad
    if (x2 is not None) != (pw.Cin2 > 0):
        raise ValueError("conv_gemm: x2 goes with weights packed by pack_weight_cat (and only with them)")
    if x2 is not None:
        _check_act(x2, "conv_gemm x2")
        if tuple(x2.shape) != (B, Hout, Wout, pw.Cin2):
            raise ValueError(f"conv_gemm: x2 shape {tuple(x2.shape)} != {(B, Hout, Wout, pw.Cin2)}")
        p.x2, p.ldx2, p.Cin2, p.cin2_pad = x2.data_ptr(), _ld(x2), pw.Cin2, pw.cin2_pad
    p.bias = None if pw.bias is None else pw.bias.data_ptr()
    if rowbias is not None:
        assert rowbias.dtype == torch.float32 and rowbias.dim() == 2 and rowbias.shape[0] == B and rowbias.stride(1) == 1
        assert rowbias.shape[1] >= pw.N
        p.rowbias, p.ld_rowbias = rowbias.data_ptr(), rowbias.stride(0)
    if colgate is not None:
        assert colgate.dtype == torch.float32 and colgate.dim() == 2 and colgate.is_contiguous()
        assert gate_group > 0 and colgate.shape[1] * gate_group == nout and B % colgate.shape[0] == 0
        p.colgate, p.gate_group, p.gate_B = colgate.data_ptr(), gate_group, colgate.shape[0]
    p.act = act
    if corr is not None:
        assert corr.dtype == torch.float32 and corr.is_contiguous() and corr.shape[1:] == (9, nout)
        assert B % corr.shape[0] == 0
        p.corr, p.corr_B = corr.data_ptr(), corr.shape[0]
    if residual is not None:
        _check_act(residual, "conv_gemm residual")
        assert tuple(residual.shape) == (B, Hout, Wout, nout)
        p.residual, p.ldres = residual.data_ptr(), _ld(residual)
    if depth is not None:
        assert depth.dtype == torch.float32 and depth.dim() == 1 and B % depth.shape[0] == 0 and depth_in is not None
        _check_act(depth_in, "conv_gemm depth_in")
        assert tuple(depth_in.shape) == (B, Hout, Wout, nout)
        p.depth, p.depth_B = depth.data_ptr(), depth.shape[0]
        p.depth_in, p.lddin = depth_in.data_ptr(), _ld(depth_in)
    p.y, p.ldy, p.out_f32 = out.data_ptr(), _ld(out), int(out_f32)
    p.epilogue = EPILOGUE
    p.io_f32 = int(f32)
    if f32:
        for t_, nm in ((x2, "x2"), (residual, "residual"), (depth_in, "depth_in")):
            if t_ is not None and t_.dtype != torch.float32:
                raise ValueError(f"conv_gemm: fp32 parity path: {nm} must be fp32 too")
    if prefetch is False:
        prefetch = None
    elif PREFETCH_WEIGHTS and prefetch is None:
        plan = _current_prefetch_plan()
        if plan is not None:
            prefetch = plan.step(pw.w)
    if prefetch is not None:
        p.prefetch, p.prefetch_bytes = prefetch.data_ptr(), prefetch.numel() * prefetch.element_size()
    plain_linear = pw.KH == 1 and pw.KW == 1 and stride == 1 and not ups and x2 is None and colgate is None and corr is None \
        and rowbias is None and depth is None and not out_f32 and gn is None and (act != ACT_GEGLU or (residual is None and not rowstats))
    p.split_k = 1
    p.tile, sk, in_kernel, p.order = choose_launch(B * Hout * Wout, pw.N, Cx, pw.cin_pad, pw.KH, pw.KW, stride, ups, act, pw.Cin2, pw.cin2_pad,
                                                   plain_linear=plain_linear, f32=f32, tile=tile, split_k=split_k, order=order)
    p.split_k = max(1, int(lib.aptp_conv_gemm_suggest_split_k(ctypes.byref(p)) if sk is None else sk))
    ws = cnt = None
    gn_fused = False
    if gn is not None and FUSE_GN_REDUCE and p.split_k > 1 and Hout * Wout <= GN_REDUCE_MAX_HW:
        gamma, beta, groups, eps_, silu_, Cn = gn
        cgn = Cn // groups
        gn_fused = Cn % 8 == 0 and Cn % groups == 0 and cgn % 4 == 0 and Hout * Wout * cgn <= 4 * 24 * 256 and Cn <= nout
    if gn_fused:
        colstats = False
        p.gn_gamma, p.gn_beta, p.gn_groups, p.gn_C, p.gn_silu, p.gn_eps = gamma.data_ptr(), beta.data_ptr(), groups, Cn, int(silu_), eps_
    want_cols = colstats and COLSTATS and Hout * Wout >= COLSTATS_MIN_HW and act != ACT_GEGLU and not out_f32
    if p.split_k > 1:
        in_kernel = splitk_in_kernel(p.split_k, in_kernel, explicit=split_k is not None, reduce_launch=gn_fused, rowstats=rowstats, colstats=want_cols)
        sk_tile = p.tile >= SK_TILE_FIRST
        if (SPLITK_IN_KERNEL or sk_tile) and (in_kernel or sk_tile) and lib.aptp_conv_gemm_tiles(ctypes.byref(p)) <= _N_COUNTERS:
            cnt = _tile_counters(x.device)
            if cnt is not None:
                p.tile_counters = cnt.data_ptr()
        if sk_tile and cnt is None:
            p.split_k = 1
        else:
            ws = _workspace(lib.aptp_conv_gemm_workspace_bytes(ctypes.byref(p)), x.device)
            p.workspace = ws.data_ptr()
    stats = None
    if rowstats and (p.split_k == 1 or cnt is not None):
        slots = lib.aptp_conv_gemm_rowstat_slots(ctypes.byref(p))
        assert slots % 2 == 0
        stats = torch.empty(slots // 2, B * Hout * Wout, 4, dtype=torch.float32, device=x.device)
        p.rowstat_out, p.rowstat_slots = stats.data_ptr(), slots
    cstats = ustat = None
    if want_cols and (p.split_k == 1 or cnt is not None) and _ld(out) % 8 == 0 and out.data_ptr() % 16 == 0 and nout % 8 == 0 \
            and (residual is None or (_ld(residual) % 8 == 0 and residual.data_ptr() % 16 == 0)) \
            and (depth_in is None or (_ld(depth_in) % 8 == 0 and depth_in.data_ptr() % 16 == 0)) and p.epilogue == 0:
        rpb = lib.aptp_conv_gemm_colstat_rows(ctypes.byref(p))
        if rpb > 0 and (Hout * Wout) % rpb == 0:
            M = B * Hout * Wout
            nblk = (M + rpb - 1) // rpb + 16
            cstats = torch.empty(nblk, nout, 2, dtype=torch.float32, device=x.device)
            p.colstat_out, p.colstat_ld = cstats.data_ptr(), nout
            ustat = _ustat_alloc(B, nout)
            if ustat is not None:
                p.ustat_out, p.ustat_unit, p.ustat_units, p.ustat_nrep = ustat[0].data_ptr(), ustat[1], ustat[2], ustat[3]
    if ln is not None:
        ln_stats, ln_eps = ln
        if pw.ln_colsum is None:
            raise ValueError("conv_gemm: ln= needs weights packed with ln_gamma / ln_beta")
        assert ln_stats.dtype == torch.float32 and ln_stats.is_contiguous() and ln_stats.shape[1] == B * Hout * Wout \
            and ln_stats.shape[2] == 4
        p.ln_stats, p.ln_slots, p.ln_colsum = ln_stats.data_ptr(), 2 * ln_stats.shape[0], pw.ln_colsum.data_ptr()
        p.ln_eps, p.ln_C = ln_eps, Cx
    elif pw.ln_colsum is not None:
        raise ValueError("conv_gemm: weights with a folded LayerNorm need ln=(stats, eps)")
    _lib.check(lib.aptp_conv_gemm(ctypes.byref(p), _stream()), "aptp_conv_gemm")
    if cstats is not None:
        _colstats_put(out, cstats, rpb, ustat)
    if LAUNCH_LOG is not None:
        LAUNCH_LOG.append({"params": p, "flops": 2.0 * B * Hout * Wout * pw.N * (pw.KH * pw.KW * pw.Cin + pw.Cin2),
                           "keep": (x, pw, out, rowbias, colgate, corr, residual, depth, depth_in, ws, stats, ln, cnt, cstats, x2, gn, ustat)})
    if f32 and gn_f32 is not None:
        gn = gn_f32
    if gn is not None and not gn_fused:
        gamma, beta, groups, eps_, silu_, Cn = gn
        return groupnorm(out, gamma, beta, groups, eps_, silu_, C=Cn)
    return (out, stats) if rowstats else out


def linear(x: torch.Tensor, pw: PackedWeight, **kw) -> torch.Tensor:
    B, L, C = x.shape
    out = kw.pop("out", None)
    for k in ("residual", "depth_in"):
        if kw.get(k) is not None:
            kw[k] = kw[k].unsqueeze(2)
    y = conv_gemm(x.unsqueeze(2), pw, pad=0, out=None if out is None else out.unsqueeze(2), **kw)
    if "rowstats" in kw:
        return (y[0].squeeze(2), y[1]) if kw["rowstats"] else (y.squeeze(2), None)
    return y.squeeze(2)


def groupnorm(x: torch.Tensor, gamma: torch.Tensor, beta: torch.Tensor, groups: int, eps: float, silu: bool,
              C: Optional[int] = None, out: Optional[torch.Tensor] = None, keep_stats: bool = False, variant: int = 0):
    lib = _lib.load()
    _check_act(x, "groupnorm x")
    B, H, W, Cp = x.shape
    C = Cp if C is None else C
    assert Cp == round_up(C, 8), f"groupnorm: tensor width {Cp} != roundup8({C})"
    assert gamma.dtype == torch.float32 and beta.dtype == torch.float32 and gamma.numel() == C and beta.numel() == C
    if out is None:
        out = torch.empty(B, H, W, Cp, dtype=x.dtype, device=x.device)
    p = GroupNormParams()
    p.x, p.ldx, p.y, p.ldy = x.data_ptr(), _ld(x), out.data_ptr(), _ld(out)
    p.B, p.HW, p.C, p.groups = B, H * W, C, groups
    p.gamma, p.beta, p.eps, p.silu = gamma.data_ptr(), beta.data_ptr(), eps, int(silu)
    if x.dtype == torch.float32:
        assert out.dtype == torch.float32 and not keep_stats
        p.io_f32, p.variant = 1, 1
        ws = _workspace(lib.aptp_groupnorm_workspace_bytes(ctypes.byref(p)), x.device)
        p.workspace = ws.data_ptr()
        _lib.check(lib.aptp_groupnorm(ctypes.byref(p), _stream()), "aptp_groupnorm(io_f32)")
        return out
    if keep_stats:
        nch = lib.aptp_groupnorm_nchunk(H * W)
        ws_full = torch.empty(B * (nch + 1) * groups * 2, dtype=torch.float32, device=x.device)
        ws = ws_full[:B * nch * groups * 2].view(B, nch, groups, 2)
        p.workspace = ws_full.data_ptr()
        p.variant = 4 if GN_STATS_ONE_LAUNCH else 1
        _lib.check(lib.aptp_groupnorm(ctypes.byref(p), _stream()), "aptp_groupnorm")
        return out, ws
    else:
        ws = _workspace(lib.aptp_groupnorm_workspace_bytes(ctypes.byref(p)), x.device)
    p.variant = variant if variant else GN_DEFAULT_VARIANT
    p.workspace = ws.data_ptr()
    segs = _colstats_get(x, C) if (COLSTATS and variant == 0 and H * W >= COLSTATS_MIN_HW) else None
    if segs is not None:
        for i, (st, rpb, cseg, us) in enumerate(segs):
            p.colstats[i].stats, p.colstats[i].ld, p.colstats[i].rows_per_block, p.colstats[i].C = st.data_ptr(), st.shape[1], rpb, cseg
            if us is not None and us[0].shape[0] == us[3] * B * us[2] * 2:
                p.colstats[i].ustats, p.colstats[i].unit, p.colstats[i].units, p.colstats[i].nrep = us[0].data_ptr(), us[1], us[2], us[3]
        p.variant = 1
    cnt = _tile_counters(x.device) if (GN_FUSED_FINALIZE and B <= _N_COUNTERS) else None
    if cnt is not None:
        p.counters = cnt.data_ptr()
    _lib.check(lib.aptp_groupnorm(ctypes.byref(p), _stream()), "aptp_groupnorm")
    if GN_LAUNCH_LOG is not None:
        GN_LAUNCH_LOG.append({"params": p, "bytes": 2.0 * B * H * W * (C + Cp), "keep": (x, out, gamma, beta, ws, segs, cnt)})
    return (out, ws) if keep_stats else out


def layernorm(x: torch.Tensor, gamma: torch.Tensor, beta: torch.Tensor, eps: float = 1e-5,
              out: Optional[torch.Tensor] = None) -> torch.Tensor:
    lib = _lib.load()
    B, L, C = x.shape
    assert x.dtype in (torch.bfloat16, torch.float32) and x.stride(2) == 1 and x.is_cuda
    ld = x.stride(1) if L > 1 else max(x.stride(1), C)
    assert B == 1 or L == 1 or x.stride(0) == L * ld
    if out is None:
        out = torch.empty(B, L, C, dtype=x.dtype, device=x.device)
    p = LayerNormParams()
    p.io_f32 = int(x.dtype == torch.float32)
    p.x, p.ldx, p.y, p.ldy = x.data_ptr(), ld, out.data_ptr(), out.stride(1) if L > 1 else C
    p.rows, p.C = B * L, C
    p.gamma, p.beta, p.eps = gamma.data_ptr(), beta.data_ptr(), eps
    _lib.check(lib.aptp_layernorm(ctypes.byref(p), _stream()), "aptp_layernorm")
    return out


def attention(q: torch.Tensor, k: torch.Tensor, v: torch.Tensor, heads: int, scale: Optional[float] = None,
              out: Optional[torch.Tensor] = None, lse: Optional[torch.Tensor] = None) -> torch.Tensor:
    lib = _lib.load()
    B, Lq = q.shape[0], q.shape[1]
    Lk = k.shape[1]
    for t in (q, k, v):
        assert t.dtype == q.dtype and t.dtype in (torch.bfloat16, torch.float32) and t.stride(2) == 1 and t.shape[2] == heads * 64 and t.is_cuda
    if out is None:
        out = torch.empty(B, Lq, heads * 64, dtype=q.dtype, device=q.device)
    p = AttentionParams()
    p.io_f32 = int(q.dtype == torch.float32)
    _set_views(p, q=q, k=k, v=v, o=out)
    p.B, p.heads, p.Lq, p.Lk = B, heads, Lq, Lk
    p.scale = (1.0 / 8.0) if scale is None else scale
    p.variant = ATTN_VARIANT
    if lse is not None:
        assert lse.dtype == torch.float32 and lse.is_contiguous() and tuple(lse.shape) == (B, heads, Lq)
        p.lse = lse.data_ptr()
    if ATTN_LAUNCH_LOG is not None and not p.io_f32:
        ATTN_LAUNCH_LOG.append({"params": p, "flops": 4.0 * B * heads * Lq * Lk * 64, "keep": (q, k, v, out, lse), "Lk": Lk})
    _lib.check(lib.aptp_attention(ctypes.byref(p), _stream()), "aptp_attention")
    return out


FUSE_GN_REDUCE = os.environ.get("APTP_FUSE_GN_REDUCE", "0") != "0"
GN_REDUCE_MAX_HW = 256


FUSE_TAIL = os.environ.get("APTP_FUSE_TAIL", "0") != "0"
FUSE_TAIL_MIN_ROWS = int(os.environ.get("APTP_FUSE_TAIL_MIN_ROWS", "16384"))


def ff_tail_supported(h: torch.Tensor, pw1: PackedWeight, pw2: PackedWeight, pw3: PackedWeight) -> bool:
    if not (FUSE_TAIL and h.is_cuda and h.dtype == torch.bfloat16 and pw1.geglu and pw1.ln_colsum is not None):
        return False
    B, L, C = h.shape
    if B * L < FUSE_TAIL_MIN_ROWS or pw2.N != C or pw3.N != C or pw2.bias is None or pw3.bias is None or pw1.bias is None:
        return False
    return bool(_lib.load().aptp_ff_tail_supported(B * L, C, pw1.N, pw1.cin_pad, pw2.cin_pad, pw3.cin_pad))


def ff_tail(h: torch.Tensor, x: torch.Tensor, pw1: PackedWeight, pw2: PackedWeight, pw3: PackedWeight, eps: float = 1e-5,
            out: Optional[torch.Tensor] = None, colstats: bool = False) -> torch.Tensor:
    lib = _lib.load()
    B, L, C = h.shape
    for t, nm in ((h, "h"), (x, "x")):
        assert t.dtype == torch.bfloat16 and t.is_cuda and tuple(t.shape) == (B, L, C) and t.stride(2) == 1, nm
    if out is None:
        out = torch.empty(B, L, C, dtype=torch.bfloat16, device=h.device)
    else:
        _colstats_drop(out.unsqueeze(2))
    assert tuple(out.shape) == (B, L, C) and out.dtype == torch.bfloat16 and out.stride(2) == 1
    p = FfTailParams()
    for name, t in (("h", h), ("x", x), ("y", out)):
        _, _, _, ld = _rows(t)
        assert B == 1 or t.stride(0) == L * ld, "rows must be uniformly strided"
        setattr(p, name, t.data_ptr())
        setattr(p, "ld" + name, ld)
    p.w1, p.b1, p.cs1, p.n1, p.ld1 = pw1.w.data_ptr(), pw1.bias.data_ptr(), pw1.ln_colsum.data_ptr(), pw1.N, pw1.cin_pad
    p.w2, p.b2, p.ld2 = pw2.w.data_ptr(), pw2.bias.data_ptr(), pw2.cin_pad
    p.w3, p.b3, p.ld3 = pw3.w.data_ptr(), pw3.bias.data_ptr(), pw3.cin_pad
    p.M, p.C, p.eps = B * L, C, eps
    cstats = None
    if colstats and COLSTATS and L >= COLSTATS_MIN_HW and L % 64 == 0:
        cstats = torch.empty(B * L // 64, C, 2, dtype=torch.float32, device=h.device)
        p.colstat, p.colstat_ld = cstats.data_ptr(), C
    _lib.check(lib.aptp_ff_tail(ctypes.byref(p), _stream()), "aptp_ff_tail")
    if cstats is not None:
        _colstats_put(out.unsqueeze(2), cstats, 64)
    if LAUNCH_LOG is not None:
        LAUNCH_LOG.append({"params": p, "fn": "aptp_ff_tail", "flops": 2.0 * B * L * (C * pw1.N + pw2.Cin * C + C * C),
                           "keep": (h, x, out, pw1, pw2, pw3, cstats)})
    return out


def unet_prologue(sample: torch.Tensor, timesteps: torch.Tensor, freqs: torch.Tensor, cin_pad: int):
    lib = _lib.load()
    assert sample.is_cuda and sample.dim() == 4 and sample.dtype in (torch.float32, torch.bfloat16)
    sample = sample.contiguous()
    B, C, H, W = sample.shape
    t = timesteps.to(device=sample.device, dtype=torch.float32).contiguous()
    assert t.numel() == B and freqs.dtype == torch.float32 and freqs.is_contiguous()
    x = torch.empty(B, H, W, cin_pad, dtype=torch.bfloat16, device=sample.device)
    temb = torch.empty(B, 2 * freqs.numel(), dtype=torch.bfloat16, device=sample.device)
    p = UnetPrologueParams()
    p.sample, p.sample_bf16, p.x = sample.data_ptr(), int(sample.dtype == torch.bfloat16), x.data_ptr()
    p.B, p.C, p.H, p.W, p.cin_pad = B, C, H, W, cin_pad
    p.timesteps, p.freqs, p.half, p.t_emb = t.data_ptr(), freqs.data_ptr(), freqs.numel(), temb.data_ptr()
    _lib.check(lib.aptp_unet_prologue(ctypes.byref(p), _stream()), "aptp_unet_prologue")
    return x, temb


def unet_epilogue(y: torch.Tensor, channels: int, out_dtype: torch.dtype, out: Optional[torch.Tensor] = None) -> torch.Tensor:
    lib = _lib.load()
    assert y.is_cuda and y.dtype == torch.float32 and y.dim() == 4 and y.is_contiguous() and out_dtype in (torch.float32, torch.bfloat16)
    B, H, W, ld = y.shape
    if out is None:
        out = torch.empty(B, channels, H, W, dtype=out_dtype, device=y.device)
    assert tuple(out.shape) == (B, channels, H, W) and out.dtype == out_dtype and out.is_contiguous() and out.is_cuda
    p = UnetEpilogueParams()
    p.y, p.ldy, p.out, p.out_bf16 = y.data_ptr(), ld, out.data_ptr(), int(out_dtype == torch.bfloat16)
    p.B, p.C, p.H, p.W = B, channels, H, W
    _lib.check(lib.aptp_unet_epilogue(ctypes.byref(p), _stream()), "aptp_unet_epilogue")
    return out


WIDE_HEAD = 512
ATTN_WIDE_LAUNCH_LOG = None


def attention_wide(q: torch.Tensor, k: torch.Tensor, v: torch.Tensor, scale: Optional[float] = None,
                   out: Optional[torch.Tensor] = None) -> torch.Tensor:
    lib = _lib.load()
    B, Lq = q.shape[0], q.shape[1]
    Lk = k.shape[1]
    for t, nm in ((q, "q"), (k, "k"), (v, "v")):
        if t.dim() != 3 or t.dtype != q.dtype or t.dtype not in (torch.bfloat16, torch.float32) or t.stride(2) != 1 \
                or t.shape[2] != WIDE_HEAD or t.shape[0] != B or not t.is_cuda:
            raise ValueError(f"attention_wide: {nm} must be a CUDA bf16 (or fp32) [B, L, 512] view with contiguous channels, "
                             f"got {t.dtype} {tuple(t.shape)} strides {t.stride()}")
    if v.shape[1] != Lk:
        raise ValueError("attention_wide: k and v must have the same length")
    if out is None:
        out = torch.empty(B, Lq, WIDE_HEAD, dtype=q.dtype, device=q.device)
    if tuple(out.shape) != (B, Lq, WIDE_HEAD) or out.dtype != q.dtype or out.stride(2) != 1:
        raise ValueError("attention_wide: out must be [B, Lq, 512] of q's dtype with contiguous channels")
    p = AttentionWideParams()
    p.io_f32 = int(q.dtype == torch.float32)
    _set_views(p, q=q, k=k, v=v, o=out)
    p.B, p.Lq, p.Lk = B, Lq, Lk
    p.scale = WIDE_HEAD ** -0.5 if scale is None else float(scale)
    if ATTN_WIDE_LAUNCH_LOG is not None and not p.io_f32:
        ATTN_WIDE_LAUNCH_LOG.append({"params": p, "flops": 4.0 * B * Lq * Lk * WIDE_HEAD, "keep": (q, k, v, out)})
    _lib.check(lib.aptp_attention_wide(ctypes.byref(p), _stream()), "aptp_attention_wide")
    return out


def image_out(y: torch.Tensor, out_dtype: torch.dtype = torch.float32, out: Optional[torch.Tensor] = None) -> torch.Tensor:
    lib = _lib.load()
    if not (y.is_cuda and y.dtype == torch.float32 and y.dim() == 4 and y.shape[3] >= 3 and y.stride(3) == 1
            and y.is_contiguous()):
        raise ValueError(f"image_out: expected a contiguous CUDA fp32 [B, H, W, >=3] tensor, got {y.dtype} {tuple(y.shape)}")
    if out_dtype not in (torch.float32, torch.uint8):
        raise ValueError("image_out: out_dtype is torch.float32 or torch.uint8")
    B, H, W, ld = y.shape
    shape = (B, H, W, 3) if out_dtype == torch.uint8 else (B, 3, H, W)
    if out is None:
        out = torch.empty(shape, dtype=out_dtype, device=y.device)
    if tuple(out.shape) != shape or out.dtype != out_dtype or not out.is_contiguous():
        raise ValueError(f"image_out: out must be a contiguous {out_dtype} {shape} tensor")
    p = ImageOutParams()
    p.y, p.ldy, p.out, p.out_u8 = y.data_ptr(), ld, out.data_ptr(), int(out_dtype == torch.uint8)
    p.B, p.H, p.W = B, H, W
    _lib.check(lib.aptp_image_out(ctypes.byref(p), _stream()), "aptp_image_out")
    return out


def image_in(x: torch.Tensor, out_f32: bool = False, out: Optional[torch.Tensor] = None) -> torch.Tensor:
    lib = _lib.load()
    if not (x.is_cuda and x.dim() == 4 and x.dtype in (torch.float32, torch.bfloat16) and x.is_contiguous()):
        raise ValueError(f"image_in: expected a contiguous CUDA fp32 / bf16 NCHW tensor, got {x.dtype} {tuple(x.shape)}")
    B, C, H, W = x.shape
    dt = torch.float32 if out_f32 else torch.bfloat16
    if out is None:
        out = torch.empty(B, H, W, 32, dtype=dt, device=x.device)
    if tuple(out.shape) != (B, H, W, 32) or out.dtype != dt or not out.is_contiguous():
        raise ValueError(f"image_in: out must be a contiguous {dt} {(B, H, W, 32)} tensor")
    p = ImageInParams()
    p.x, p.x_bf16, p.out, p.out_f32 = x.data_ptr(), int(x.dtype == torch.bfloat16), out.data_ptr(), int(out_f32)
    p.B, p.C, p.H, p.W = B, C, H, W
    _lib.check(lib.aptp_image_in(ctypes.byref(p), _stream()), "aptp_image_in")
    return out


def pack_conv_in_im2col(w: torch.Tensor, bias: Optional[torch.Tensor], device=None) -> PackedWeight:
    O, C, KH, KW = w.shape
    if (C, KH, KW) != (3, 3, 3):
        raise ValueError(f"pack_conv_in_im2col: expected a [O, 3, 3, 3] weight, got {tuple(w.shape)}")
    w2 = torch.zeros(O, 32, dtype=torch.float32, device=w.device)
    w2[:, :27] = w.detach().float().permute(0, 2, 3, 1).reshape(O, 27)
    return pack_weight(w2, None if bias is None else bias.detach(), device=device)


def latent_dist(y: torch.Tensor, wq: torch.Tensor, bq: torch.Tensor, eps: Optional[torch.Tensor] = None,
                scale: float = 1.0, moments: bool = True, latents_dtype: torch.dtype = torch.float32,
                moments_out: Optional[torch.Tensor] = None, latents_out: Optional[torch.Tensor] = None):
    lib = _lib.load()
    if not (y.is_cuda and y.dtype == torch.float32 and y.dim() == 4 and y.shape[3] >= 8 and y.is_contiguous()):
        raise ValueError(f"latent_dist: expected a contiguous CUDA fp32 [B, h, w, >=8] tensor, got {y.dtype} {tuple(y.shape)}")
    B, H, W, ld = y.shape
    wq = wq.to(device=y.device, dtype=torch.float32).reshape(8, 8).contiguous()
    bq = bq.to(device=y.device, dtype=torch.float32).reshape(8).contiguous()
    p = LatentDistParams()
    p.y, p.ldy, p.wq, p.bq = y.data_ptr(), ld, wq.data_ptr(), bq.data_ptr()
    p.B, p.H, p.W, p.scale = B, H, W, float(scale)
    mom = lat = None
    if moments:
        mom = moments_out if moments_out is not None else torch.empty(B, 8, H, W, dtype=torch.float32, device=y.device)
        if tuple(mom.shape) != (B, 8, H, W) or mom.dtype != torch.float32 or not mom.is_contiguous():
            raise ValueError(f"latent_dist: moments must be a contiguous fp32 {(B, 8, H, W)} tensor")
        p.moments = mom.data_ptr()
    if eps is not None:
        if tuple(eps.shape) != (B, 4, H, W) or eps.dtype != torch.float32 or not eps.is_contiguous() or eps.device != y.device:
            raise ValueError(f"latent_dist: eps must be a contiguous fp32 {(B, 4, H, W)} tensor on {y.device}")
        if latents_dtype not in (torch.float32, torch.bfloat16):
            raise ValueError("latent_dist: latents_dtype is torch.float32 or torch.bfloat16")
        lat = latents_out if latents_out is not None else torch.empty(B, 4, H, W, dtype=latents_dtype, device=y.device)
        if tuple(lat.shape) != (B, 4, H, W) or lat.dtype != latents_dtype or not lat.is_contiguous():
            raise ValueError(f"latent_dist: latents must be a contiguous {latents_dtype} {(B, 4, H, W)} tensor")
        p.eps, p.latents, p.latents_bf16 = eps.data_ptr(), lat.data_ptr(), int(latents_dtype == torch.bfloat16)
    _lib.check(lib.aptp_latent_dist(ctypes.byref(p), _stream()), "aptp_latent_dist")
    return mom, lat


CAUSAL_MAX_L = 128


def attention_causal(q: torch.Tensor, k: torch.Tensor, v: torch.Tensor, heads: int, scale: Optional[float] = None,
                     out: Optional[torch.Tensor] = None) -> torch.Tensor:
    lib = _lib.load()
    B, L = q.shape[0], q.shape[1]
    if out is None:
        out = torch.empty(B, L, heads * 64, dtype=q.dtype, device=q.device)
    _check_heads64_views(q, k, v, out, B, L, heads, "attention_causal")
    p = AttentionCausalParams()
    p.io_f32 = int(q.dtype == torch.float32)
    _set_views(p, q=q, k=k, v=v, o=out)
    p.B, p.heads, p.L = B, heads, L
    p.scale = 0.125 if scale is None else scale
    _lib.check(lib.aptp_attention_causal(ctypes.byref(p), _stream()), "aptp_attention_causal")
    return out


def token_embed(ids: torch.Tensor, tok: torch.Tensor, pos: torch.Tensor, out_f32: bool = False,
                out: Optional[torch.Tensor] = None) -> torch.Tensor:
    lib = _lib.load()
    if ids.dtype != torch.int64 or ids.dim() != 2 or not ids.is_contiguous() or not ids.is_cuda:
        raise ValueError(f"token_embed: ids must be a contiguous CUDA int64 [B, L] tensor, got {ids.dtype} {tuple(ids.shape)}")
    B, L = ids.shape
    V, C = tok.shape
    for t, nm in ((tok, "tok"), (pos, "pos")):
        if t.dtype != torch.float32 or t.dim() != 2 or not t.is_contiguous() or t.shape[1] != C or t.device != ids.device:
            raise ValueError(f"token_embed: {nm} must be a contiguous fp32 [rows, {C}] tensor on the ids' device")
    if pos.shape[0] < L:
        raise ValueError(f"token_embed: {L} tokens but only {pos.shape[0]} positions")
    odt = torch.float32 if out_f32 else torch.bfloat16
    if out is None:
        out = torch.empty(B, L, C, dtype=odt, device=ids.device)
    elif tuple(out.shape) != (B, L, C) or out.dtype != odt or not out.is_contiguous():
        raise ValueError(f"token_embed: out must be a contiguous {odt} [{B}, {L}, {C}] tensor")
    p = TokenEmbedParams()
    p.ids, p.tok, p.pos, p.out, p.ldo = ids.data_ptr(), tok.data_ptr(), pos.data_ptr(), out.data_ptr(), C
    p.B, p.L, p.C, p.vocab, p.out_f32, p.pos_rows = B, L, C, V, int(out_f32), pos.shape[0]
    _lib.check(lib.aptp_token_embed(ctypes.byref(p), _stream()), "aptp_token_embed")
    return out


BIAS_MAX_L = 512


def _check_heads64_views(q, k, v, out, B: int, L: int, heads: int, name: str):
    for t in (q, k, v, out):
        if t.dtype != q.dtype or t.dtype not in (torch.bfloat16, torch.float32) or t.dim() != 3 or t.stride(2) != 1 \
                or tuple(t.shape) != (B, L, heads * 64) or not t.is_cuda or t.device != q.device:
            raise ValueError(f"{name}: q, k, v and out must be {q.dtype} [B, L, {heads * 64}] views with contiguous "
                             f"channels on {q.device}, got {t.dtype} {tuple(t.shape)} strides {t.stride()} on {t.device}")


def _check_mask(mask: Optional[torch.Tensor], B: int, L: int, device, name: str):
    if mask is not None and (mask.dtype != torch.float32 or tuple(mask.shape) != (B, L) or not mask.is_contiguous()
                             or mask.device != device):
        raise ValueError(f"{name}: the mask must be a contiguous fp32 [{B}, {L}] tensor on {device}, got {mask.dtype} "
                         f"{tuple(mask.shape)} on {mask.device}")


def attention_bias(q: torch.Tensor, k: torch.Tensor, v: torch.Tensor, heads: int, relbias: torch.Tensor,
                   key_mask: Optional[torch.Tensor] = None, scale: Optional[float] = None,
                   out: Optional[torch.Tensor] = None) -> torch.Tensor:
    lib = _lib.load()
    B, L = q.shape[0], q.shape[1]
    if out is None:
        out = torch.empty(B, L, heads * 64, dtype=q.dtype, device=q.device)
    _check_heads64_views(q, k, v, out, B, L, heads, "attention_bias")
    if relbias.dtype != torch.float32 or tuple(relbias.shape) != (heads, 2 * L - 1) or not relbias.is_contiguous() \
            or relbias.device != q.device:
        raise ValueError(f"attention_bias: relbias must be a contiguous fp32 [{heads}, {2 * L - 1}] tensor on {q.device}, got "
                         f"{relbias.dtype} {tuple(relbias.shape)} on {relbias.device}")
    _check_mask(key_mask, B, L, q.device, "attention_bias")
    p = AttentionBiasParams()
    p.io_f32 = int(q.dtype == torch.float32)
    _set_views(p, q=q, k=k, v=v, o=out)
    p.relbias, p.key_mask = relbias.data_ptr(), (None if key_mask is None else key_mask.data_ptr())
    p.B, p.heads, p.L = B, heads, L
    p.scale = 0.125 if scale is None else scale
    _lib.check(lib.aptp_attention_bias(ctypes.byref(p), _stream()), "aptp_attention_bias")
    return out


def embed_ln(ids: torch.Tensor, word: torch.Tensor, pos: torch.Tensor, gamma: torch.Tensor, beta: torch.Tensor,
             eps: float = 1e-5, pad_id: int = 1, out_f32: bool = False, out: Optional[torch.Tensor] = None) -> torch.Tensor:
    lib = _lib.load()
    if ids.dtype != torch.int64 or ids.dim() != 2 or not ids.is_contiguous() or not ids.is_cuda:
        raise ValueError(f"embed_ln: ids must be a contiguous CUDA int64 [B, L] tensor, got {ids.dtype} {tuple(ids.shape)}")
    B, L = ids.shape
    V, C = word.shape
    for t, nm, shp in ((word, "word", (V, C)), (pos, "pos", (pos.shape[0], C)), (gamma, "gamma", (C,)), (beta, "beta", (C,))):
        if t.dtype != torch.float32 or tuple(t.shape) != shp or not t.is_contiguous() or t.device != ids.device:
            raise ValueError(f"embed_ln: {nm} must be a contiguous fp32 {shp} tensor on the ids' device")
    if pos.shape[0] <= L + pad_id:
        raise ValueError(f"embed_ln: {L} tokens with pad id {pad_id} need {L + pad_id + 1} positions, have {pos.shape[0]}")
    odt = torch.float32 if out_f32 else torch.bfloat16
    if out is None:
        out = torch.empty(B, L, C, dtype=odt, device=ids.device)
    elif tuple(out.shape) != (B, L, C) or out.dtype != odt or not out.is_contiguous():
        raise ValueError(f"embed_ln: out must be a contiguous {odt} [{B}, {L}, {C}] tensor")
    p = EmbedLnParams()
    p.ids, p.word, p.pos, p.gamma, p.beta = ids.data_ptr(), word.data_ptr(), pos.data_ptr(), gamma.data_ptr(), beta.data_ptr()
    p.out, p.ldo = out.data_ptr(), C
    p.B, p.L, p.C, p.vocab, p.pos_rows, p.pad_id, p.out_f32, p.eps = B, L, C, V, pos.shape[0], pad_id, int(out_f32), eps
    _lib.check(lib.aptp_embed_ln(ctypes.byref(p), _stream()), "aptp_embed_ln")
    return out


def masked_mean(x: torch.Tensor, mask: Optional[torch.Tensor] = None, out: Optional[torch.Tensor] = None) -> torch.Tensor:
    lib = _lib.load()
    if x.dtype not in (torch.bfloat16, torch.float32) or x.dim() != 3 or x.stride(2) != 1 or not x.is_cuda:
        raise ValueError(f"masked_mean: x must be a CUDA bf16 or fp32 [B, L, C] tensor with contiguous channels, got {x.dtype} "
                         f"{tuple(x.shape)}")
    B, L, C = x.shape
    _check_mask(mask, B, L, x.device, "masked_mean")
    if out is None:
        out = torch.empty(B, C, dtype=torch.float32, device=x.device)
    elif tuple(out.shape) != (B, C) or out.dtype != torch.float32 or not out.is_contiguous() or out.device != x.device:
# ... 1176 lines not shown
```

### diffusion_pruning_amd/unet.py

```python
from __future__ import annotations

import os

import math
from dataclasses import dataclass, field
from typing import Any, Dict, List, Optional, Tuple, Union

import torch
import torch.nn as nn

from . import ops
from .gates import DepthGate, LinearWidthGate, WidthGate
from .modules import LinearP, PlannedModule, _capturing, _Params, _PlanCache, _versions
from .ops import PackedWeight



class Conv2dP(_Params):
    def __init__(self, cin, cout, k):
        super().__init__()
        self.in_channels, self.out_channels, self.kernel_size = cin, cout, (k, k)
        self.weight = nn.Parameter(torch.empty(cout, cin, k, k))
        self.bias = nn.Parameter(torch.empty(cout))

# ... 1118 lines not shown
    def from_config(cls, config: Optional[dict] = None, **kwargs):
        cfg = dict(config or {})
        cfg.update(kwargs)
        return cls(**cfg)

    @torch.no_grad()
    def init_synthetic(self, seed: int = 0, w_std: float = 0.02, beta_std: float = 0.1):
        g = torch.Generator().manual_seed(seed)
        for name, prm in self.named_parameters():
            owner = self.get_submodule(name.rsplit(".", 1)[0])
            if isinstance(owner, NormP):
                if name.endswith(".weight"):
                    prm.fill_(1.0)
                else:
                    prm.copy_(torch.randn(prm.shape, generator=g) * beta_std)
            elif name.endswith(".weight"):
                prm.copy_(torch.randn(prm.shape, generator=g) * w_std)
            else:
                prm.copy_(torch.randn(prm.shape, generator=g) * (0.5 * w_std))
        self.invalidate_plans()
        return self

    def invalidate_plans(self):
        self._misc.clear()
        self._batched.clear()
        for m in self.modules():
            if m is not self and hasattr(m, "invalidate"):
                m.invalidate()

    def _apply(self, fn, *a, **k):
        out = super()._apply(fn, *a, **k)
        self.invalidate_plans()
        return out

    def load_state_dict(self, *a, **k):
        out = super().load_state_dict(*a, **k)
        self.invalidate_plans()
        return out

    def state_dict(self, *a, **k):
        pk = self.__dict__.get("_pk")
        if pk is not None:
            pk.export_()
        return super().state_dict(*a, **k)

    def save_pretrained(self, save_directory: str, **unused):
        from . import checkpoint
        root, sub = os.path.split(os.path.normpath(save_directory))
        checkpoint.save_pretrained(self, root, subfolder=sub)

    @classmethod
    def from_pretrained(cls, pretrained_model_name_or_path: str, subfolder: Optional[str] = None, **kwargs):
        from . import checkpoint
        return checkpoint.from_pretrained(pretrained_model_name_or_path, subfolder=subfolder, cls=cls, **kwargs)

    def freeze(self):
        for name, param in self.named_parameters():
            if "gate_f" not in name:
                param.requires_grad = False

    def _containers(self):
        return list(self.down_blocks) + [self.mid_block] + list(self.up_blocks)

    def get_structure(self):
        if len(self.structure["width"]) == 0:
            structure = {"width": [], "depth": []}
            for m in self._containers():
                s = m.get_gate_structure()
                assert len(s) == 2 and len(s["width"]) == len(s["depth"])
                structure["width"] = structure["width"] + s["width"]
                structure["depth"] = structure["depth"] + s["depth"]
            self.structure = structure
        return self.structure

    def set_structure(self, arch_vectors, prefetch_hosts: bool = True):
        width_vectors, depth_vectors = arch_vectors["width"], arch_vectors["depth"]
        self._installed_structure = {"width": list(width_vectors), "depth": list(depth_vectors)}
        self._structure_epoch = self.__dict__.get("_structure_epoch", 0) + 1
        self._host_map = {}
        if prefetch_hosts:
            self._prefetch_hosts(width_vectors, depth_vectors)
        for m in self._containers():
            s = m.get_gate_structure()
            block_vectors = {"width": [], "depth": []}
            for i in range(len(s["width"])):
                for j in range(len(s["width"][i])):
                    assert s["width"][i][j] == width_vectors[0].shape[1]
                    block_vectors["width"].append(width_vectors.pop(0))
            for i in range(len(s["depth"])):
                if s["depth"][i] == [1]:
                    block_vectors["depth"].append(depth_vectors.pop(0))
            m.set_gate_structure(block_vectors)
        self._attach_hosts()

    def _prefetch_hosts(self, width_vectors, depth_vectors):
        self._host_map = {}
        tensors = list(width_vectors) + list(depth_vectors)
        if not tensors:
            return
        if all(t.device.type == "cpu" for t in tensors):
            return
        flat = torch.cat([t.detach().float().reshape(-1) for t in tensors]).cpu()
        off = 0
        for t in tensors:
            n = t.numel()
            self._host_map[id(t)] = flat[off:off + n].reshape(t.shape)
            off += n

    def _attach_hosts(self):
        hm = getattr(self, "_host_map", None)
        if not hm:
            return
        for m in self.modules():
            if isinstance(m, (WidthGate, DepthGate)):
                h = hm.get(id(m.gate_f))
                if h is not None:
                    m.set_host_value(h)
        self._host_map = {}

    def count_macs(self, latent_h: int, latent_w: Optional[int] = None, text_len: int = 77):
        from . import macs
        macs.assign_module_macs(self, latent_h, latent_w, text_len)
        sanity = self.calc_macs()
        self.prunable_macs_list = [[e / sanity["prunable_macs"] for e in elem] for elem in self.get_prunable_macs()]
        self.resource_info_dict = sanity
        return sanity

    def calc_macs(self):
        from . import macs
        return macs.unet_calc_macs(self)

    def get_prunable_macs(self):
        from . import macs
        return macs.unet_get_prunable_macs(self)

    def get_block_utilization(self):
        from . import macs
        return macs.unet_get_block_utilization(self)

    def _resnets(self):
        return [m for m in self.modules() if isinstance(m, ResnetBlock2DWidthGated)]

    def _transformers(self):
        return [m for m in self.modules() if isinstance(m, Transformer2DModelWidthGated)]

    def _misc_packs(self, dev):
        ver = () if self.__dict__.get("_pk") is not None else \
            tuple(p._version for mod in (self.conv_in, self.time_embedding, self.conv_norm_out, self.conv_out) for p in mod.parameters())
        m = self._misc.get(str(dev), ver)
        if m is None:
            cin_pad = ops.round_up(self.in_channels, 8)
            m = {"cin_pad": cin_pad}
            m["conv_in"] = ops.pack_weight(self.conv_in.weight.detach(), self.conv_in.bias.detach(), device=dev)
            te = self.time_embedding
            m["t1"] = ops.pack_weight(te.linear_1.weight.detach(), te.linear_1.bias.detach(), device=dev)
            m["t2"] = ops.pack_weight(te.linear_2.weight.detach(), te.linear_2.bias.detach(), device=dev)
            m["gn_g"], m["gn_b"] = _f32(self.conv_norm_out.weight).to(dev), _f32(self.conv_norm_out.bias).to(dev)
            m["conv_out"] = ops.pack_weight(self.conv_out.weight.detach(), self.conv_out.bias.detach(), device=dev)
            half = self.conv_in.out_channels // 2
            m["freqs"] = torch.exp(-math.log(10000.0) * torch.arange(half, dtype=torch.float32, device=dev) / half)
            self._misc.put(str(dev), ver, m)
        return m

    def _batched_packs(self, dev):
        resnets, trans = self._resnets(), self._transformers()
        for r in resnets:
            r.semantics = self.semantics
        rplans = [r.plan(dev) for r in resnets if not (r.depth_gated and (r.dropped or r._depth_state()[0] == 0.0))]
        live_res = [r for r in resnets if not (r.depth_gated and (r.dropped or r._depth_state()[0] == 0.0))]
        live_tr = [t for t in trans if not (t.depth_gated and (t.dropped or t._depth_state()[0] == 0.0))]
        tplans = [t.plan(dev) for t in live_tr]
        key = (tuple(id(p) for p in rplans), tuple(id(p) for p in tplans), str(dev))
        bp = self._batched.get(key, ())
        if bp is not None:
            return bp
        bp = {"key": key, "plans": (rplans, tplans)}
        ws, bs, slots, off = [], [], [], 0
        for r, pl in zip(live_res, rplans):
            npad = pl["c_pad"]
            w, b = pl["temb_w"], pl["temb_b"]
            if w.shape[0] != npad:
                w = torch.cat([w, w.new_zeros(npad - w.shape[0], w.shape[1])], 0)
                b = torch.cat([b, b.new_zeros(npad - b.shape[0])], 0)
            ws.append(w); bs.append(b)
            slots.append((id(r), off, npad))
            off += npad
        bp["temb_pw"] = ops.pack_weight(torch.cat(ws, 0), torch.cat(bs, 0), device=dev)
        bp["temb_slots"] = slots
        ws, slots, off, gates = [], [], 0, []
        for t, pl in zip(live_tr, tplans):
            w = pl["a2_kv_w"]
            ws.append(w)
            slots.append((id(t.transformer_blocks[0].attn2), off, w.shape[0]))
            off += w.shape[0]
            gates.append((t.transformer_blocks[0].attn2.gate, pl["a2_dense_gate"], pl["a2_heads"]))
        if ws:
            bp["kv_pw"] = ops.pack_weight(torch.cat(ws, 0), None, device=dev)
        bp["kv_slots"] = slots
        bp["kv_gates"] = gates
        return self._batched.put(key, (), bp)

    def _project_context(self, encoder_hidden_states, bp, dev) -> CtxBundle:
        ehs = encoder_hidden_states.to(device=dev, dtype=ops.ACT_DTYPE).contiguous()
        reusable = not any(dense for (_, dense, _) in bp["kv_gates"])
        ctx = CtxBundle(ehs=ehs, key=bp["key"] if reusable else None)
        if bp["kv_slots"]:
            gkw = {}
            if any(dense for (_, dense, _) in bp["kv_gates"]):
                cols = []
                for gate, dense, hl in bp["kv_gates"]:
                    g = gate.gate_f.detach().to(device=dev, dtype=torch.float32) if dense else None
                    bg = max(gt.gate_f.shape[0] for gt, d_, _ in bp["kv_gates"] if d_)
                    if g is None:
                        g = torch.ones(bg, hl, device=dev)
                    elif g.shape[0] != bg:
                        g = g.repeat(bg // g.shape[0], 1)
                    cols.append(g.repeat(1, 2))
                gkw = dict(colgate=torch.cat(cols, 1).contiguous(), gate_group=64)
            kv_all = ops.linear(ehs, bp["kv_pw"], **gkw)
            for aid, off, n in bp["kv_slots"]:
                ctx.kv[aid] = kv_all[..., off:off + n]
        return ctx

    @torch.no_grad()
    def precompute_context(self, encoder_hidden_states: torch.Tensor) -> CtxBundle:
        dev = encoder_hidden_states.device
        return self._project_context(encoder_hidden_states, self._batched_packs(dev), dev)

    def _register_cat_slots(self, B, H, W, c_in, dev):
        if _ft_mode(self):
            return None
        skips = [None]
        for blk in self.down_blocks:
            for i in range(len(blk.resnets)):
                skips.append(blk.attentions[i] if blk.has_cross_attention else blk.resnets[i])
            if blk.downsamplers is not None:
                skips.append(blk.downsamplers[0])
        prev = self.mid_block.resnets[-1]
        conv_in_slot = None
        for blk in self.up_blocks:
            for i, resnet in enumerate(blk.resnets):
                cs = resnet.skip_connection_dim
                slot = _CatSlot(resnet.in_channels - cs, cs)
                prev.__dict__["_out_dst"] = (slot, 0)
                sk = skips.pop()
                if sk is None:
                    conv_in_slot = slot
                else:
                    sk.__dict__["_out_dst"] = (slot, 1)
                prev = blk.attentions[i] if blk.has_cross_attention else resnet
            if blk.upsamplers is not None:
                prev = blk.upsamplers[0]
        return None if conv_in_slot is None else conv_in_slot.view(1, B, H, W, c_in, dev)

    def _forward_ft(self, sample, timestep, encoder_hidden_states, return_dict):
        from . import autograd as AG
        dev = sample.device
        B = sample.shape[0]
        misc = self._misc_packs(dev)
        for r in self._resnets():
            r.semantics = self.semantics

        def bwd(name, param):
            def get():
                if name not in misc:
                    misc[name] = ops.pack_weight_dgrad(param.detach(), device=dev)
                return misc[name]
            return get
        timesteps = timestep
        if not torch.is_tensor(timesteps):
            timesteps = torch.tensor([timesteps], dtype=torch.int64, device=dev)
        elif timesteps.dim() == 0:
            timesteps = timesteps[None].to(dev)
        timesteps = timesteps.to(dev).expand(B)
        ang = timesteps.float()[:, None] * misc["freqs"][None, :]
        t_emb = torch.cat([torch.cos(ang), torch.sin(ang)], dim=-1).to(torch.bfloat16)
        te = self.time_embedding
        e1 = _cw(self, t_emb[None], te.linear_1.weight, te.linear_1.bias, misc["t1"], bwd("t1_bwd", te.linear_1.weight), pad=0, out_f32=True)
        e1 = torch.nn.functional.silu(e1).to(torch.bfloat16)
        e2 = _cw(self, e1, te.linear_2.weight, te.linear_2.bias, misc["t2"], bwd("t2_bwd", te.linear_2.weight), pad=0, out_f32=True)
        temb = TembBundle(emb_silu=torch.nn.functional.silu(e2)[0].to(torch.bfloat16))
        ctx = CtxBundle(ehs=encoder_hidden_states.to(device=dev, dtype=torch.bfloat16).contiguous())
        x = torch.zeros(B, sample.shape[2], sample.shape[3], misc["cin_pad"], dtype=torch.bfloat16, device=dev)
        x[..., :self.in_channels] = sample.permute(0, 2, 3, 1)
        live_in = torch.arange(self.in_channels, device=dev)
        h = _nchw(_cw(self, x, self.conv_in.weight, self.conv_in.bias, misc["conv_in"], bwd("conv_in_bwd", self.conv_in.weight),
                            live_in=live_in))
        res_samples = (h,)
        for blk in self.down_blocks:
            h, res = blk(hidden_states=h, temb=temb, encoder_hidden_states=ctx)
            res_samples += res
        h = self.mid_block(h, temb, encoder_hidden_states=ctx)
        for blk in self.up_blocks:
            n_res = len(blk.resnets)
            res = res_samples[-n_res:]
            res_samples = res_samples[:-n_res]
            h = blk(hidden_states=h, temb=temb, res_hidden_states_tuple=res, encoder_hidden_states=ctx)
        a = _gnw(self, _nhwc(h), self.conv_norm_out.weight, self.conv_norm_out.bias, misc["gn_g"], misc["gn_b"],
                                  self.conv_norm_out.num_groups, self.conv_norm_out.eps, True, self.conv_norm_out.num_channels, None)
        live_out = torch.arange(self.out_channels, device=dev)
        y = _cw(self, a, self.conv_out.weight, self.conv_out.bias, misc["conv_out"], bwd("conv_out_bwd", self.conv_out.weight),
                      out_f32=True, live_out=live_out)
        out = y[..., :self.out_channels].permute(0, 3, 1, 2).to(sample.dtype)
        if not return_dict:
            return (out,)
        return UNet2DConditionOutput(sample=out)

    def forward(self, sample: torch.Tensor, timestep, encoder_hidden_states: torch.Tensor, class_labels=None,
                timestep_cond=None, attention_mask=None, cross_attention_kwargs=None, added_cond_kwargs=None,
                down_block_additional_residuals=None, mid_block_additional_residual=None, encoder_attention_mask=None,
                return_dict: bool = True):
        if attention_mask is not None or encoder_attention_mask is not None or class_labels is not None \
                or down_block_additional_residuals is not None or mid_block_additional_residual is not None:
            raise NotImplementedError("only the arguments the APTP trainer/pipeline pass are supported")
        dev = sample.device
        B = sample.shape[0]
        plans = self.__dict__.setdefault("_pf_plans", {})
        mode = torch.is_grad_enabled()
        if mode not in plans:
            plans[mode] = ops._PrefetchPlan()
        ops.set_prefetch_plan(plans[mode])
        if not mode and sample.is_cuda:
            unit = self.__dict__.get("_ustat_unit")
            if unit is None:
                import math
                g = self.conv_norm_out.num_groups
                unit = 0
                for c in self.config["block_out_channels"]:
                    unit = math.gcd(unit, c // g) if c % g == 0 else 1
                unit = self.__dict__["_ustat_unit"] = unit if unit >= 4 else 0
            ops.ustat_begin(dev, unit)
        try:
            return self._forward_impl(sample, timestep, encoder_hidden_states, return_dict)
        finally:
            ops.set_prefetch_plan(None)
            ops.ustat_end()

    def _forward_impl(self, sample, timestep, encoder_hidden_states, return_dict):
        dev = sample.device
        B = sample.shape[0]
        if _ft_mode(self) and self.conv_in.weight.requires_grad:
            return self._forward_ft(sample, timestep, encoder_hidden_states, return_dict)
        misc = self._misc_packs(dev)
        bp = self._batched_packs(dev)
        out_dtype = sample.dtype

        timesteps = timestep
        if not torch.is_tensor(timesteps):
            timesteps = torch.tensor([timesteps], dtype=torch.int64, device=dev)
        elif timesteps.dim() == 0:
            timesteps = timesteps[None].to(dev)
        timesteps = timesteps.to(dev).expand(B)
        fused_io = sample.is_cuda and sample.dtype in (torch.float32, torch.bfloat16) and not torch.is_grad_enabled() \
            and ops.ACT_DTYPE == torch.bfloat16
        if fused_io:
            x, t_emb = ops.unet_prologue(sample, timesteps, misc["freqs"], misc["cin_pad"])
        else:
            ang = timesteps.float()[:, None] * misc["freqs"][None, :]
            t_emb = torch.cat([torch.cos(ang), torch.sin(ang)], dim=-1).to(ops.ACT_DTYPE)
            x = None
        e1 = ops.linear(t_emb[None], misc["t1"], act=ops.ACT_SILU)
        emb_silu = ops.linear(e1, misc["t2"], act=ops.ACT_SILU)
        tproj = ops.linear(emb_silu, bp["temb_pw"], out_f32=True)[0]
        temb = TembBundle(emb_silu=emb_silu[0])
        for rid, off, npad in bp["temb_slots"]:
            temb.proj[rid] = tproj[:, off:off + npad]

        if isinstance(encoder_hidden_states, CtxBundle) and encoder_hidden_states.key is not None \
                and encoder_hidden_states.key == bp["key"]:
            ctx = encoder_hidden_states
        else:
            ehs_in = encoder_hidden_states.ehs if isinstance(encoder_hidden_states, CtxBundle) else encoder_hidden_states
            ctx = self._project_context(ehs_in, bp, dev)

        if x is None:
            x = torch.zeros(B, sample.shape[2], sample.shape[3], misc["cin_pad"], dtype=ops.ACT_DTYPE, device=dev)
            x[..., :self.in_channels] = sample.permute(0, 2, 3, 1)
        conv_in_dst = self._register_cat_slots(B, x.shape[1], x.shape[2], misc["conv_in"].N, dev)
        h = _nchw(ops.conv_gemm(x, misc["conv_in"], out=conv_in_dst, colstats=True))

        down_block_res_samples = (h,)
        for blk in self.down_blocks:
            h, res = blk(hidden_states=h, temb=temb, encoder_hidden_states=ctx)
            down_block_res_samples += res
        h = self.mid_block(h, temb, encoder_hidden_states=ctx)
        for blk in self.up_blocks:
            n_res = len(blk.resnets)
            res = down_block_res_samples[-n_res:]
            down_block_res_samples = down_block_res_samples[:-n_res]
            h = blk(hidden_states=h, temb=temb, res_hidden_states_tuple=res, encoder_hidden_states=ctx)
        if torch.is_grad_enabled() and h.requires_grad:
            from . import autograd as AG

            def get_out_bwd():
                if "conv_out_bwd" not in misc:
                    misc["conv_out_bwd"] = ops.pack_weight_dgrad(self.conv_out.weight.detach(), device=dev)
                return misc["conv_out_bwd"]
            a = AG.GroupNormFn.apply(_nhwc(h), misc["gn_g"], misc["gn_b"], self.conv_norm_out.num_groups, self.conv_norm_out.eps, True)
            y = AG.conv(a, misc["conv_out"], get_out_bwd, out_f32=True)
        else:
            a = ops.groupnorm(_nhwc(h), misc["gn_g"], misc["gn_b"], self.conv_norm_out.num_groups, self.conv_norm_out.eps, True)
            y = ops.conv_gemm(a, misc["conv_out"], out_f32=True)
            if fused_io:
                out = ops.unet_epilogue(y, self.out_channels, out_dtype)
                return (out,) if not return_dict else UNet2DConditionOutput(sample=out)
        out = y[..., :self.out_channels].permute(0, 3, 1, 2).to(out_dtype)
        if not return_dict:
            return (out,)
        return UNet2DConditionOutput(sample=out)


class UNet2DConditionModelPruned(UNet2DConditionModelGated):

    def __init__(self, *args, **kwargs):
        super().__init__(*args, **kwargs)
        self.semantics = "pruned"

    def load_state_dict(self, state_dict, strict: bool = True, **k):
        own = self.state_dict()
        full = all(kk in state_dict and tuple(state_dict[kk].shape) == tuple(v.shape) for kk, v in own.items())
        if full or not getattr(self, "_installed_structure", None):
            return super().load_state_dict(state_dict, strict=strict, **k)
        from . import checkpoint
        return checkpoint.load_pruned_state_dict(self, state_dict, strict=strict)

    def prune(self, arch_vectors):
        hard = {"width": [(w.detach() >= 0.5).float() for w in arch_vectors["width"]],
                "depth": [(d.detach() >= 0.5).float() for d in arch_vectors["depth"]]}
        for t in hard["width"] + hard["depth"]:
            assert t.shape[0] == 1, "Pruning is only supported for single batch size"
        self.set_structure(hard)
        for r in self._resnets():
            r.pruned = True
            r.dropped = bool(r.depth_gated and r._depth_state()[0] == 0.0)
        for t in self._transformers():
            t.pruned = True
            t.dropped = bool(t.depth_gated and t._depth_state()[0] == 0.0)
        return self
```

### include/aptp_hip.h

```cpp
#ifndef APTP_HIP_H
#define APTP_HIP_H

#include <stdint.h>

#ifdef __cplusplus
extern "C" {
#endif

typedef void* aptp_stream_t;

enum {
  APTP_OK = 0,
  APTP_EINVAL = -1,
  APTP_ELAUNCH = -2,
  APTP_EWORKSPACE = -3
};

enum { APTP_ACT_NONE = 0, APTP_ACT_SILU = 1, APTP_ACT_GEGLU = 2, APTP_ACT_GELU = 3, APTP_ACT_QUICK_GELU = 5 };

typedef struct {
  const void* x;
  int64_t ldx;
  int32_t B, Hin, Win, Cin;
  int32_t Hout, Wout;
  int32_t KH, KW, stride, pad, ups;
  const void* w;
  int32_t N;
  int32_t cin_pad;
  const float* bias;
  const float* rowbias;
  int32_t ld_rowbias;
  const float* colgate;
  int32_t gate_group, gate_B;
  int32_t act;
  const float* corr;
  int32_t corr_B;
  const void* residual;
  int64_t ldres;
  const float* depth;
  int32_t depth_B;
  const void* depth_in;
  int64_t lddin;
  void* y;
  int64_t ldy;
  int32_t out_f32;
  int32_t split_k;
  void* workspace;
  int32_t tile;
  int32_t order;
  float* rowstat_out;
  int32_t rowstat_slots;
  const float* ln_stats;
  int32_t ln_slots;
  const float* ln_colsum;
  float ln_eps;
  int32_t ln_C;
  float* colstat_out;
  int32_t colstat_ld;
  int32_t* tile_counters;
  const void* x2;
  int64_t ldx2;
  int32_t Cin2, cin2_pad;
  const void* prefetch;
  int64_t prefetch_bytes;
  int32_t epilogue;
  const float* gn_gamma;
  const float* gn_beta;
  int32_t gn_groups, gn_C, gn_silu;
  float gn_eps;
  int32_t io_f32;
  void* ustat_out;
  int32_t ustat_unit, ustat_units, ustat_nrep;
  int32_t pad_end;
} AptpConvGemmParams;

enum { APTP_TILE_AUTO = 0, APTP_TILE_128x128 = 1, APTP_TILE_128x160 = 2, APTP_TILE_64x128 = 3, APTP_TILE_64x160 = 4,
       APTP_TILE_128x64 = 5, APTP_TILE_64x64 = 6,
       APTP_TILE_DMA_128x128 = 7, APTP_TILE_DMA_128x160 = 8, APTP_TILE_DMA_64x128 = 9, APTP_TILE_DMA_64x160 = 10,
       APTP_TILE_DMA_128x64 = 11, APTP_TILE_DMA_64x64 = 12,
       APTP_TILE_DMA3_128x128 = 13, APTP_TILE_DMA3_128x160 = 14, APTP_TILE_DMA3_64x128 = 15, APTP_TILE_DMA3_64x160 = 16,
       APTP_TILE_DMA3_128x64 = 17, APTP_TILE_DMA3_64x64 = 18,
       APTP_TILE_DMA8_128x160 = 19, APTP_TILE_DMA8_256x160 = 20, APTP_TILE_DMA8_128x128 = 21, APTP_TILE_DMA8_256x128 = 22,
       APTP_TILE_DMA4_64x160 = 23, APTP_TILE_DMA4_64x128 = 24, APTP_TILE_DMA4_64x64 = 25, APTP_TILE_DMA4_128x64 = 26,
       APTP_TILE_DMA4_128x128 = 27,
       APTP_TILE_DMA8R3_128x160 = 28, APTP_TILE_DMA8R4_128x160 = 29, APTP_TILE_DMA8R3_128x128 = 30,
       APTP_TILE_DMA8R4_128x128 = 31, APTP_TILE_DMA8R3_256x128 = 32,
       APTP_TILE_PP3_128x160 = 33, APTP_TILE_PP4_128x160 = 34, APTP_TILE_PP3_128x128 = 35, APTP_TILE_PP4_128x128 = 36,
       APTP_TILE_PP4_64x160 = 37, APTP_TILE_PP4_64x128 = 38, APTP_TILE_PP5_64x160 = 39, APTP_TILE_PP4_128x64 = 40,
       APTP_TILE_PP3_256x128 = 41, APTP_TILE_PP3_128x256 = 42,
       APTP_TILE_HALO_128x160 = 43, APTP_TILE_HALO_128x128 = 44,
       APTP_TILE_DMA6_64x64 = 45, APTP_TILE_DMA8S_64x64 = 46, APTP_TILE_DMA6_64x128 = 47, APTP_TILE_DMA6_128x64 = 48,
       APTP_TILE_KU2S4_64x64 = 49, APTP_TILE_KU2S6_64x64 = 50, APTP_TILE_KU2S4_64x128 = 51, APTP_TILE_KU2S6_64x128 = 52,
       APTP_TILE_KU2S4_128x64 = 53, APTP_TILE_KU2S4_128x128 = 54, APTP_TILE_KU2S4_64x160 = 55, APTP_TILE_KU2S4_128x160 = 56,
       APTP_TILE_KU2S4_128x128W8 = 57,
       APTP_TILE_KS2S3_64x64 = 58, APTP_TILE_KS2S4_64x64 = 59, APTP_TILE_KS2S3_64x128 = 60, APTP_TILE_KS2S4_64x128 = 61,
       APTP_TILE_KS2S3_128x64 = 62, APTP_TILE_KS2S3_128x128 = 63,
       APTP_TILE_SK_256x160 = 64, APTP_TILE_SK_256x128 = 65, APTP_TILE_SK_128x256 = 66,
       APTP_TILE_SKL_256x160 = 67, APTP_TILE_SKL_256x128 = 68, APTP_TILE_SKL_128x256 = 69,
       APTP_TILE_SK_128x160 = 70, APTP_TILE_SKL_128x160 = 71, APTP_TILE_SK_128x128 = 72, APTP_TILE_SKL_128x128 = 73 };

int aptp_conv_gemm(const AptpConvGemmParams* p, aptp_stream_t stream);
int64_t aptp_conv_gemm_workspace_bytes(const AptpConvGemmParams* p);
int aptp_conv_gemm_colstat_rows(const AptpConvGemmParams* p);
int aptp_conv_gemm_tiles(const AptpConvGemmParams* p);
int aptp_conv_gemm_rowstat_slots(const AptpConvGemmParams* p);
int aptp_conv_gemm_suggest_split_k(const AptpConvGemmParams* p);

typedef struct {
  const float* stats;
  int32_t ld, rows_per_block, C;
  const void* ustats;
  int32_t unit, units, nrep;
} AptpGroupNormColStats;

typedef struct {
  const void* x; int64_t ldx;
  void* y; int64_t ldy;
  int32_t B, HW, C, groups;
  const float* gamma; const float* beta;
  float eps;
  int32_t silu;
  void* workspace;
  int32_t variant;
  int32_t* counters;
  AptpGroupNormColStats colstats[2];
  int32_t io_f32;
} AptpGroupNormParams;

int aptp_groupnorm(const AptpGroupNormParams* p, aptp_stream_t stream);
int aptp_groupnorm_nchunk(int HW);
int aptp_rows_nchunk(int rows);
int64_t aptp_groupnorm_workspace_bytes(const AptpGroupNormParams* p);

typedef struct {
  const void* x; int64_t ldx;
  void* y; int64_t ldy;
  int32_t rows, C;
  const float* gamma; const float* beta;
  float eps;
  int32_t io_f32;
} AptpLayerNormParams;

int aptp_layernorm(const AptpLayerNormParams* p, aptp_stream_t stream);

typedef struct {
  const void* q; int64_t q_stride_b, q_stride_l;
  const void* k; int64_t k_stride_b, k_stride_l;
  const void* v; int64_t v_stride_b, v_stride_l;
  void* o; int64_t o_stride_b, o_stride_l;
  int32_t B, heads, Lq, Lk;
  float scale;
  float* lse;
  int32_t variant;
  int32_t io_f32;
} AptpAttentionParams;

int aptp_attention(const AptpAttentionParams* p, aptp_stream_t stream);

typedef struct {
  const void* sample; int32_t sample_bf16;
  void* x;
  int32_t B, C, H, W, cin_pad;
  const float* timesteps;
  const float* freqs;
  int32_t half;
  void* t_emb;
} AptpUnetPrologueParams;

typedef struct {
  const float* y; int64_t ldy;
  void* out; int32_t out_bf16;
  int32_t B, C, H, W;
} AptpUnetEpilogueParams;

int aptp_unet_prologue(const AptpUnetPrologueParams* p, aptp_stream_t stream);
int aptp_unet_epilogue(const AptpUnetEpilogueParams* p, aptp_stream_t stream);

typedef struct {
  const void* q; int64_t q_stride_b, q_stride_l;
  const void* k; int64_t k_stride_b, k_stride_l;
  const void* v; int64_t v_stride_b, v_stride_l;
  void* o; int64_t o_stride_b, o_stride_l;
  int32_t B, Lq, Lk;
  float scale;
  int32_t io_f32;
} AptpAttentionWideParams;

int aptp_attention_wide(const AptpAttentionWideParams* p, aptp_stream_t stream);

typedef struct {
  const float* y; int64_t ldy;
  void* out; int32_t out_u8;
  int32_t B, H, W;
} AptpImageOutParams;

int aptp_image_out(const AptpImageOutParams* p, aptp_stream_t stream);

typedef struct {
  const void* x; int32_t x_bf16;
  void* out; int32_t out_f32;
  int32_t B, C, H, W;
} AptpImageInParams;

int aptp_image_in(const AptpImageInParams* p, aptp_stream_t stream);

typedef struct {
  const float* y; int64_t ldy;
  const float* wq;
  const float* bq;
  float* moments;
  const float* eps;
  void* latents; int32_t latents_bf16;
  float scale;
  int32_t B, H, W;
} AptpLatentDistParams;

int aptp_latent_dist(const AptpLatentDistParams* p, aptp_stream_t stream);

typedef struct {
  const void* q; int64_t q_stride_b, q_stride_l;
  const void* k; int64_t k_stride_b, k_stride_l;
  const void* v; int64_t v_stride_b, v_stride_l;
  void* o; int64_t o_stride_b, o_stride_l;
  int32_t B, heads, L;
  float scale;
  int32_t io_f32;
} AptpAttentionCausalParams;

int aptp_attention_causal(const AptpAttentionCausalParams* p, aptp_stream_t stream);

typedef struct {
  const int64_t* ids;
  const float* tok;
  const float* pos;
  void* out; int64_t ldo;
  int32_t B, L, C, vocab;
  int32_t out_f32;
  int32_t pos_rows;
} AptpTokenEmbedParams;

int aptp_token_embed(const AptpTokenEmbedParams* p, aptp_stream_t stream);

typedef struct {
  const void* q; int64_t q_stride_b, q_stride_l;
  const void* k; int64_t k_stride_b, k_stride_l;
  const void* v; int64_t v_stride_b, v_stride_l;
  void* o; int64_t o_stride_b, o_stride_l;
  const float* relbias;
  const float* key_mask;
  int32_t B, heads, L;
  float scale;
  int32_t io_f32;
} AptpAttentionBiasParams;

int aptp_attention_bias(const AptpAttentionBiasParams* p, aptp_stream_t stream);

typedef struct {
  const int64_t* ids;
  const float* word;
  const float* pos;
  const float* gamma;
  const float* beta;
  void* out; int64_t ldo;
  int32_t B, L, C, vocab;
  int32_t pos_rows;
  int32_t pad_id;
  int32_t out_f32;
  float eps;
} AptpEmbedLnParams;

int aptp_embed_ln(const AptpEmbedLnParams* p, aptp_stream_t stream);

typedef struct {
  const void* x; int64_t x_stride_b, x_stride_l;
  const float* mask;
  float* out;
  int32_t B, L, C;
  int32_t x_f32;
} AptpMaskedMeanParams;

int aptp_masked_mean(const AptpMaskedMeanParams* p, aptp_stream_t stream);

typedef struct {
  const void* h; int64_t ldh;
  const void* x; int64_t ldx;
  void* y; int64_t ldy;
  const void* w1; const float* b1; const float* cs1; int32_t n1, ld1;
  const void* w2; const float* b2; int32_t ld2;
  const void* w3; const float* b3; int32_t ld3;
  float* colstat; int32_t colstat_ld;
  int32_t M, C;
  float eps;
} AptpFfTailParams;
int aptp_ff_tail_supported(int M, int C, int n1, int ld1, int ld2, int ld3);
int aptp_ff_tail(const AptpFfTailParams* p, aptp_stream_t stream);


typedef struct {
  const void* dy; int64_t lddy;
  const void* y0; int64_t ldy0;
  void* dx; int64_t lddx;
  int32_t B, HW, C, groups;
  const float* gate; int32_t gate_B;
  float* dgate_partial;
  float* dgate;
} AptpGateBwdParams;
int aptp_gate_bwd(const AptpGateBwdParams* p, aptp_stream_t stream);

typedef struct {
  const void* hg; int64_t ldhg;
  void* out; int64_t ldout;
  const void* dout; int64_t lddout;
  void* dhg; int64_t lddhg;
  int32_t B, HW, C, groups;
  const float* gate; int32_t gate_B;
  float* dgate_partial;
  int32_t backward;
  float* dgate;
} AptpGegluParams;
int aptp_geglu(const AptpGegluParams* p, aptp_stream_t stream);

typedef struct {
  const void* x_in; int64_t ld_in;
  const void* x_out; int64_t ld_out;
  void* y; int64_t ld_y;
  const void* dy; int64_t ld_dy;
  void* d_in; int64_t ld_d_in;
  void* d_out; int64_t ld_d_out;
  int32_t B, HW, C;
// ... 268 lines not shown
```

Before: 205.3 steps/s.

## Fuse U-Net head work into prologue and add skinny GEMV path for tiny linears

Adds a skinny GEMV kernel that handles linears with at most 8 rows (time-embedding MLP, per-block temb projections) in place of the tiled conv GEMM. It also extends the U-Net prologue kernel to do several things in one launch: read int64 timesteps directly, zero the deferred ustat arena, cast fp32 encoder hidden states to bf16, and emit an im2col layout so conv_in runs as a K=64 GEMM. The aim is to cut small-kernel launch count and the poor tile utilisation of tiny-M GEMMs at the head of the forward pass. In exchange there are more code paths and extra env-gated branches, and the new epilogue-3 marker only changes routing when HEAD_TAIL is off.

```diff
diff --git a/diffusion_pruning_amd/_lib.py b/diffusion_pruning_amd/_lib.py
--- a/diffusion_pruning_amd/_lib.py
+++ b/diffusion_pruning_amd/_lib.py
@@ -202,6 +202,8 @@
         ("sample", c_void_p), ("sample_bf16", c_int32), ("x", c_void_p),
         ("B", c_int32), ("C", c_int32), ("H", c_int32), ("W", c_int32), ("cin_pad", c_int32),
         ("timesteps", c_void_p), ("freqs", c_void_p), ("half", c_int32), ("t_emb", c_void_p),
+        ("timesteps_i64", c_int32), ("timesteps_stride", c_int64), ("zero", c_void_p), ("zero_bytes", c_int64),
+        ("cast_src", c_void_p), ("cast_dst", c_void_p), ("cast_n", c_int64), ("im2col", c_int32),
     ]
 
 
@@ -209,6 +211,14 @@
     _fields_ = [
         ("y", c_void_p), ("ldy", c_int64), ("out", c_void_p), ("out_bf16", c_int32),
         ("B", c_int32), ("C", c_int32), ("H", c_int32), ("W", c_int32),
+    ]
+
+
+class LinSkinnyParams(Structure):
+    _fields_ = [
+        ("x", c_void_p), ("ldx", c_int64), ("w", c_void_p), ("ldw", c_int64), ("bias", c_void_p),
+        ("y", c_void_p), ("ldy", c_int64),
+        ("M", c_int32), ("N", c_int32), ("K", c_int32), ("act", c_int32), ("out_f32", c_int32),
     ]
 
 
@@ -525,6 +535,9 @@
     ("aptp_layernorm_pgrad", c_int, [POINTER(LayerNormPgradParams), c_void_p]),
     ("aptp_unet_prologue", c_int, [POINTER(UnetPrologueParams), c_void_p]),
     ("aptp_unet_epilogue", c_int, [POINTER(UnetEpilogueParams), c_void_p]),
+    ("aptp_lin_skinny", c_int, [POINTER(LinSkinnyParams), c_void_p]),
+    ("aptp_lin_skinny_supported", c_int, [POINTER(LinSkinnyParams)]),
+    ("aptp_conv_gemm_is_skinny", c_int, [POINTER(ConvGemmParams)]),
     ("aptp_attention_wide", c_int, [POINTER(AttentionWideParams), c_void_p]),
     ("aptp_image_out", c_int, [POINTER(ImageOutParams), c_void_p]),
     ("aptp_image_in", c_int, [POINTER(ImageInParams), c_void_p]),
diff --git a/diffusion_pruning_amd/csrc/conv_gemm.hip b/diffusion_pruning_amd/csrc/conv_gemm.hip
--- a/diffusion_pruning_amd/csrc/conv_gemm.hip
+++ b/diffusion_pruning_amd/csrc/conv_gemm.hip
@@ -1133,10 +1133,30 @@
   return s < 1 ? 1 : s;
 }
 
+static bool skinny_params(const AptpConvGemmParams* p, AptpLinSkinnyParams& q) {
+  if (p->epilogue != 0 || p->io_f32 || p->KH != 1 || p->KW != 1 || p->stride != 1 || p->pad != 0 || p->ups != 0 || p->pad_end != 0) return false;
+  if (p->x2 || p->rowbias || p->colgate || p->corr || p->residual || p->depth || p->rowstat_out || p->colstat_out || p->ln_stats ||
+      p->gn_gamma || p->ustat_out) return false;
+  const int64_t M = (int64_t)p->B * p->Hout * p->Wout;
+  if (M > 8) return false;
+  q.x = p->x; q.ldx = p->ldx; q.w = p->w; q.ldw = p->cin_pad; q.bias = p->bias; q.y = p->y; q.ldy = p->ldy;
+  q.M = (int)M; q.N = p->N; q.K = p->Cin; q.act = p->act; q.out_f32 = p->out_f32;
+  return aptp_lin_skinny_supported(&q) != 0;
+}
+
+extern "C" int aptp_conv_gemm_is_skinny(const AptpConvGemmParams* p) {
+  AptpLinSkinnyParams q;
+  return p && skinny_params(p, q) ? 1 : 0;
+}
+
 extern "C" int aptp_conv_gemm(const AptpConvGemmParams* p, aptp_stream_t stream) {
   KParams k;
   const int rc = fill_kparams(p, k);
   if (rc != APTP_OK) return rc;
+  {
+    AptpLinSkinnyParams q;
+    if (skinny_params(p, q)) return aptp_lin_skinny(&q, stream);
+  }
   if (k.split_k > 1) APTP_CHECK(k.ws != nullptr && ((uintptr_t)k.ws % 16) == 0, "conv_gemm: split_k > 1 needs a 16B-aligned workspace");
   if (k.split_k == 1) k.counters = nullptr;
   k.gn_gamma = p->gn_gamma; k.gn_beta = p->gn_beta; k.gn_groups = p->gn_groups; k.gn_C = p->gn_C; k.gn_silu = p->gn_silu; k.gn_eps = p->gn_eps;
@@ -1192,14 +1212,15 @@
     k.fd_perm = make_fastdiv(tiles_n * k.split_k); k.fd_tmn = make_fastdiv(tiles_m * tiles_n);
   }
   static const bool lin_on = !(getenv("APTP_LIN") && getenv("APTP_LIN")[0] == '0');
-  if (lin_on && p->epilogue != 2 && p->pad_end == 0 && aptp_lin_eligible(k, t)) {
+  const int epi = p->epilogue == 3 ? 0 : p->epilogue;
+  if (lin_on && epi != 2 && p->pad_end == 0 && aptp_lin_eligible(k, t)) {
     const int rc2 = aptp_launch_lin(k, t, s);
     if (rc2 != APTP_OK) return rc2;
     APTP_LAUNCH_CHECK();
     return APTP_OK;
   }
   static const bool lean_on = !(getenv("APTP_CONV_LEAN") && getenv("APTP_CONV_LEAN")[0] == '0');
-  if (lean_on && p->epilogue == 0 && p->pad_end == 0 && aptp_conv_lean_eligible(k, t)) {
+  if (lean_on && epi == 0 && p->pad_end == 0 && aptp_conv_lean_eligible(k, t)) {
     const int rc2 = aptp_launch_conv_lean(k, t, s);
     if (rc2 != APTP_OK) return rc2;
   } else
diff --git a/diffusion_pruning_amd/csrc/lin_skinny.hip b/diffusion_pruning_amd/csrc/lin_skinny.hip
--- /dev/null
+++ b/diffusion_pruning_amd/csrc/lin_skinny.hip
@@ -0,0 +1,131 @@
+#include "aptp_common.h"
+
+namespace {
+
+constexpr int NCH = 4;
+
+struct SkK {
+  const __bf16* x; int64_t ldx;
+  const __bf16* w; int64_t ldw;
+  const float* bias;
+  void* y; int64_t ldy;
+  int M, N, KC;
+  int act, out_f32;
+  int lgG, passes, iters;
+};
+
+template <int MT>
+__global__ __launch_bounds__(256) void lin_skinny_kernel(const SkK p) {
+  extern __shared__ uint4 xs[];
+  const int tid = threadIdx.x, lane = tid & 63, wave = tid >> 6;
+  const int KC = p.KC;
+  for (int i = tid; i < MT * KC; i += 256) {
+    const int m = i / KC, kc = i - m * KC;
+    uint4 v = make_uint4(0u, 0u, 0u, 0u);
+    if (m < p.M) v = *reinterpret_cast<const uint4*>(p.x + (int64_t)m * p.ldx + (int64_t)kc * 8);
+    xs[i] = v;
+  }
+  __syncthreads();
+  const int G = 1 << p.lgG, sub = lane & (G - 1), cg = lane >> p.lgG, cpw = 64 >> p.lgG;
+  const int64_t g0 = ((int64_t)blockIdx.x * 4 + wave) * p.iters;
+  const int steps = p.iters * p.passes;
+
+  auto issue = [&](int s, uint4 (&wv)[NCH]) {
+    const int it = s / p.passes, ps = s - it * p.passes;
+    const int64_t col = (g0 + it) * cpw + cg;
+    const __bf16* row = p.w + col * p.ldw;
+#pragma unroll
+    for (int j = 0; j < NCH; ++j) {
+      const int kc = (ps * NCH + j) * G + sub;
+      wv[j] = make_uint4(0u, 0u, 0u, 0u);
+      if (col < p.N && kc < KC) wv[j] = *reinterpret_cast<const uint4*>(row + (int64_t)kc * 8);
+    }
+  };
+
+  float acc[MT];
+#pragma unroll
+  for (int m = 0; m < MT; ++m) acc[m] = 0.f;
+  uint4 wn[NCH];
+  issue(0, wn);
+  for (int s = 0; s < steps; ++s) {
+    uint4 wc[NCH];
+#pragma unroll
+    for (int j = 0; j < NCH; ++j) wc[j] = wn[j];
+    if (s + 1 < steps) issue(s + 1, wn);
+    const int it = s / p.passes, ps = s - it * p.passes;
+#pragma unroll
+    for (int j = 0; j < NCH; ++j) {
+      const int kc = (ps * NCH + j) * G + sub;
+      if (kc < KC) {
+        float wf[8];
+        unpack_bf16x8(wc[j], wf);
+#pragma unroll
+        for (int m = 0; m < MT; ++m) {
+          float xf[8];
+          unpack_bf16x8(xs[m * KC + kc], xf);
+#pragma unroll
+          for (int e = 0; e < 8; ++e) acc[m] = __builtin_fmaf(wf[e], xf[e], acc[m]);
+        }
+      }
+    }
+    if (ps + 1 < p.passes) continue;
+    for (int off = G >> 1; off; off >>= 1) {
+#pragma unroll
+      for (int m = 0; m < MT; ++m) acc[m] += __shfl_xor(acc[m], off, 64);
+    }
+    const int64_t col = (g0 + it) * cpw + cg;
+    if (col < p.N) {
+      const float b = p.bias ? p.bias[col] : 0.f;
+#pragma unroll
+      for (int m = 0; m < MT; ++m) {
+        if (m < p.M && sub == (m & (G - 1))) {
+          float v = acc[m] + b;
+          if (p.act == APTP_ACT_SILU) v = silu_f(v);
+          if (p.out_f32) reinterpret_cast<float*>(p.y)[(int64_t)m * p.ldy + col] = v;
+          else reinterpret_cast<__bf16*>(p.y)[(int64_t)m * p.ldy + col] = (__bf16)v;
+        }
+      }
+    }
+#pragma unroll
+    for (int m = 0; m < MT; ++m) acc[m] = 0.f;
+  }
+}
+
+}
+
+extern "C" int aptp_lin_skinny_supported(const AptpLinSkinnyParams* p) {
+  return p && p->M >= 1 && p->M <= 8 && p->N >= 1 && p->K >= 8 && p->K % 8 == 0 && p->K <= 4096 &&
+         (p->act == APTP_ACT_NONE || p->act == APTP_ACT_SILU) ? 1 : 0;
+}
+
+extern "C" int aptp_lin_skinny(const AptpLinSkinnyParams* p, aptp_stream_t stream) {
+  APTP_CHECK(p && p->x && p->w && p->y, "lin_skinny: null pointer");
+  APTP_CHECK(aptp_lin_skinny_supported(p), "lin_skinny: needs 1 <= M <= 8, N >= 1, K a multiple of 8 in [8, 4096], act none / SiLU "
+             "(got M %d N %d K %d act %d)", p->M, p->N, p->K, p->act);
+  APTP_CHECK(p->ldx >= p->K && p->ldx % 8 == 0 && p->ldw >= p->K && p->ldw % 8 == 0 && p->ldy >= p->N,
+             "lin_skinny: ldx, ldw must be multiples of 8 and >= K, ldy >= N");
+  APTP_CHECK(((uintptr_t)p->x % 16) == 0 && ((uintptr_t)p->w % 16) == 0 && ((uintptr_t)p->y % (p->out_f32 ? 4 : 2)) == 0 &&
+             ((uintptr_t)p->bias % 4) == 0, "lin_skinny: pointer alignment");
+  SkK k;
+  k.x = reinterpret_cast<const __bf16*>(p->x); k.ldx = p->ldx;
+  k.w = reinterpret_cast<const __bf16*>(p->w); k.ldw = p->ldw;
+  k.bias = p->bias; k.y = p->y; k.ldy = p->ldy;
+  k.M = p->M; k.N = p->N; k.KC = p->K / 8; k.act = p->act; k.out_f32 = p->out_f32 ? 1 : 0;
+  int lg = 2;
+  while (lg < 6 && (NCH << lg) < k.KC) ++lg;
+  k.lgG = lg;
+  k.passes = (k.KC + (NCH << lg) - 1) / (NCH << lg);
+  const int cpw = 64 >> lg;
+  const int64_t groups = ((int64_t)p->N + cpw - 1) / cpw;
+  int64_t iters = groups / (4 * 512);
+  iters = iters < 1 ? 1 : (iters > 8 ? 8 : iters);
+  k.iters = (int)iters;
+  const int64_t blocks = (groups + 4 * iters - 1) / (4 * iters);
+  APTP_CHECK(blocks < (1ll << 31), "lin_skinny: N too large");
+  const int mt = p->M <= 4 ? 4 : 8;
+  const size_t lds = (size_t)mt * k.KC * sizeof(uint4);
+  if (mt == 4) hipLaunchKernelGGL(lin_skinny_kernel<4>, dim3((unsigned)blocks), dim3(256), lds, (hipStream_t)stream, k);
+  else hipLaunchKernelGGL(lin_skinny_kernel<8>, dim3((unsigned)blocks), dim3(256), lds, (hipStream_t)stream, k);
+  APTP_LAUNCH_CHECK();
+  return APTP_OK;
+}
diff --git a/diffusion_pruning_amd/csrc/unet_io.hip b/diffusion_pruning_amd/csrc/unet_io.hip
--- a/diffusion_pruning_amd/csrc/unet_io.hip
+++ b/diffusion_pruning_amd/csrc/unet_io.hip
@@ -3,17 +3,53 @@
 namespace {
 
 struct IoK {
-  const void* sample; int sample_bf16; void* x; int B, C, HW, cpad;
-  const float* t; const float* freqs; int half; void* temb;
-  int pix_blocks;
+  const void* sample; int sample_bf16; void* x; int B, C, H, W, HW, cpad;
+  const void* t; int t_i64; int64_t t_stride; const float* freqs; int half; void* temb;
+  uint4* zero; int64_t zero_q;
+  const float* cast_src; uint4* cast_dst; int64_t cast_q;
+  int im2col;
+  int pix_blocks, t_blocks, zero_blocks;
 };
+
+constexpr int IM2COL_K = 64;
+constexpr int ZERO_PER_THREAD = 4;
 
 __global__ __launch_bounds__(256) void unet_prologue_kernel(const IoK p) {
   const int tid = threadIdx.x;
-  if ((int)blockIdx.x < p.pix_blocks) {
-    const int64_t pix = (int64_t)blockIdx.x * 256 + tid;
+  int blk = (int)blockIdx.x;
+  if (blk < p.pix_blocks) {
+    const int64_t pix = (int64_t)blk * 256 + tid;
     if (pix >= (int64_t)p.B * p.HW) return;
     const int b = (int)(pix / p.HW), r = (int)(pix - (int64_t)b * p.HW);
+    if (p.im2col) {
+      const int oy = r / p.W, ox = r - oy * p.W;
+      float v[40];
+#pragma unroll
+      for (int e = 36; e < 40; ++e) v[e] = 0.f;
+#pragma unroll
+      for (int ky = 0; ky < 3; ++ky) {
+#pragma unroll
+        for (int kx = 0; kx < 3; ++kx) {
+          const int iy = oy + ky - 1, ix = ox + kx - 1;
+          const bool ok = (unsigned)iy < (unsigned)p.H && (unsigned)ix < (unsigned)p.W;
+#pragma unroll
+          for (int c = 0; c < 4; ++c) {
+            float f = 0.f;
+            if (ok) {
+              const int64_t i = ((int64_t)b * 4 + c) * p.HW + (int64_t)iy * p.W + ix;
+              f = p.sample_bf16 ? (float)reinterpret_cast<const __bf16*>(p.sample)[i] : reinterpret_cast<const float*>(p.sample)[i];
+            }
+            v[(ky * 3 + kx) * 4 + c] = f;
+          }
+        }
+      }
+      uint4* dst = reinterpret_cast<uint4*>(reinterpret_cast<__bf16*>(p.x) + pix * IM2COL_K);
+#pragma unroll
+      for (int q = 0; q < 5; ++q) dst[q] = pack_bf16x8(v + 8 * q);
+#pragma unroll
+      for (int q = 5; q < IM2COL_K / 8; ++q) dst[q] = make_uint4(0u, 0u, 0u, 0u);
+      return;
+    }
     __bf16* dst = reinterpret_cast<__bf16*>(p.x) + pix * p.cpad;
     for (int c0 = 0; c0 < p.cpad; c0 += 8) {
       float f[8];
@@ -31,13 +67,33 @@
     }
     return;
   }
-  const int i = ((int)blockIdx.x - p.pix_blocks) * 256 + tid;
-  if (i >= p.B * p.half) return;
-  const int b = i / p.half, k = i - b * p.half;
-  const float a = p.t[b] * p.freqs[k];
-  __bf16* e = reinterpret_cast<__bf16*>(p.temb) + (int64_t)b * 2 * p.half;
-  e[k] = (__bf16)cosf(a);
-  e[p.half + k] = (__bf16)sinf(a);
+  blk -= p.pix_blocks;
+  if (blk < p.t_blocks) {
+    const int i = blk * 256 + tid;
+    if (i >= p.B * p.half) return;
+    const int b = i / p.half, k = i - b * p.half;
+    const float t = p.t_i64 ? (float)reinterpret_cast<const int64_t*>(p.t)[(int64_t)b * p.t_stride] : reinterpret_cast<const float*>(p.t)[b];
+    const float a = t * p.freqs[k];
+    __bf16* e = reinterpret_cast<__bf16*>(p.temb) + (int64_t)b * 2 * p.half;
+    e[k] = (__bf16)cosf(a);
+    e[p.half + k] = (__bf16)sinf(a);
+    return;
+  }
+  blk -= p.t_blocks;
+  if (blk < p.zero_blocks) {
+#pragma unroll
+    for (int j = 0; j < ZERO_PER_THREAD; ++j) {
+      const int64_t q = ((int64_t)blk * ZERO_PER_THREAD + j) * 256 + tid;
+      if (q < p.zero_q) p.zero[q] = make_uint4(0u, 0u, 0u, 0u);
+    }
+    return;
+  }
+  blk -= p.zero_blocks;
+  const int64_t q = (int64_t)blk * 256 + tid;
+  if (q >= p.cast_q) return;
+  const float4 a = reinterpret_cast<const float4*>(p.cast_src)[2 * q], c = reinterpret_cast<const float4*>(p.cast_src)[2 * q + 1];
+  const float f[8] = {a.x, a.y, a.z, a.w, c.x, c.y, c.z, c.w};
+  p.cast_dst[q] = pack_bf16x8(f);
 }
 
 struct OutK { const float* y; int64_t ld; void* out; int out_bf16; int B, C, HW; };
@@ -234,13 +290,29 @@
   APTP_CHECK(p->B > 0 && p->C > 0 && p->H > 0 && p->W > 0 && p->cin_pad >= p->C && p->cin_pad % 8 == 0 && p->half > 0,
              "unet_prologue: bad extents (cin_pad must be a multiple of 8 and >= C)");
   APTP_CHECK(((uintptr_t)p->x % 16) == 0, "unet_prologue: x alignment");
+  APTP_CHECK(!p->im2col || p->C == 4, "unet_prologue: the im2col form is built for C = 4 (got %d)", p->C);
+  APTP_CHECK(((uintptr_t)p->timesteps % (p->timesteps_i64 ? 8 : 4)) == 0 && (!p->timesteps_i64 || p->timesteps_stride >= 0),
+             "unet_prologue: timesteps alignment / stride");
+  APTP_CHECK(p->zero_bytes >= 0 && p->zero_bytes % 16 == 0 && (p->zero_bytes == 0 || (p->zero && ((uintptr_t)p->zero % 16) == 0)),
+             "unet_prologue: zero range must be 16-byte aligned and a multiple of 16 bytes");
+  APTP_CHECK(p->cast_n >= 0 && p->cast_n % 8 == 0 &&
+             (p->cast_n == 0 || (p->cast_src && p->cast_dst && ((uintptr_t)p->cast_src % 16) == 0 && ((uintptr_t)p->cast_dst % 16) == 0)),
+             "unet_prologue: cast range must be 16-byte aligned and a multiple of 8 elements");
   IoK k;
-  k.sample = p->sample; k.sample_bf16 = p->sample_bf16; k.x = p->x; k.B = p->B; k.C = p->C; k.HW = p->H * p->W; k.cpad = p->cin_pad;
-  k.t = p->timesteps; k.freqs = p->freqs; k.half = p->half; k.temb = p->t_emb;
+  k.sample = p->sample; k.sample_bf16 = p->sample_bf16; k.x = p->x; k.B = p->B; k.C = p->C; k.H = p->H; k.W = p->W; k.HW = p->H * p->W;
+  k.cpad = p->cin_pad;
+  k.t = p->timesteps; k.t_i64 = p->timesteps_i64 ? 1 : 0; k.t_stride = p->timesteps_stride; k.freqs = p->freqs; k.half = p->half;
+  k.temb = p->t_emb;
+  k.zero = reinterpret_cast<uint4*>(p->zero); k.zero_q = p->zero_bytes / 16;
+  k.cast_src = p->cast_src; k.cast_dst = reinterpret_cast<uint4*>(p->cast_dst); k.cast_q = p->cast_n / 8;
+  k.im2col = p->im2col ? 1 : 0;
   const int64_t pix = (int64_t)p->B * k.HW;
   k.pix_blocks = (int)((pix + 255) / 256);
-  const int tblocks = (p->B * p->half + 255) / 256;
-  hipLaunchKernelGGL(unet_prologue_kernel, dim3(k.pix_blocks + tblocks), dim3(256), 0, (hipStream_t)stream, k);
+  k.t_blocks = (p->B * p->half + 255) / 256;
+  const int64_t zb = (k.zero_q + 256 * ZERO_PER_THREAD - 1) / (256 * ZERO_PER_THREAD), cb = (k.cast_q + 255) / 256;
+  APTP_CHECK((int64_t)p->H * p->W < (1ll << 31) && (pix + 255) / 256 + k.t_blocks + zb + cb < (1ll << 31), "unet_prologue: too much work for one launch");
+  k.zero_blocks = (int)zb;
+  hipLaunchKernelGGL(unet_prologue_kernel, dim3((unsigned)(k.pix_blocks + k.t_blocks + zb + cb)), dim3(256), 0, (hipStream_t)stream, k);
   APTP_LAUNCH_CHECK();
   return APTP_OK;
 }
diff --git a/diffusion_pruning_amd/ops.py b/diffusion_pruning_amd/ops.py
--- a/diffusion_pruning_amd/ops.py
+++ b/diffusion_pruning_amd/ops.py
@@ -270,21 +270,30 @@
 _ustat_arenas = {}
 
 
-def ustat_begin(device, unit: int):
+def ustat_begin(device, unit: int, defer: bool = False):
     if not USTAT or unit <= 0 or torch.device(device).type != "cuda":
         _tls.ustat = None
         return
     capturing = torch.cuda.is_current_stream_capturing()
     key = (torch.device(device).index, torch.cuda.current_stream().cuda_stream, _domain(), capturing)
+    defer = defer and HEAD_TAIL
+    pending = 0
     ent = _ustat_arenas.get(key)
     if ent is None:
-        ent = _ustat_arenas[key] = {"buf": torch.zeros(_USTAT_WORDS, dtype=torch.int64, device=device), "used": 0}
+        if capturing and defer:
+            ent = _ustat_arenas[key] = {"buf": torch.empty(_USTAT_WORDS, dtype=torch.int64, device=device), "used": 0}
+            pending = _USTAT_WORDS
+        else:
+            ent = _ustat_arenas[key] = {"buf": torch.zeros(_USTAT_WORDS, dtype=torch.int64, device=device), "used": 0}
         if capturing:
             _ws_capture_keep.append(ent["buf"])
             ent["used"] = _USTAT_WORDS
     elif ent["used"]:
-        ent["buf"][:ent["used"]].zero_()
-    _tls.ustat = {"buf": ent["buf"], "off": 0, "unit": int(unit), "ent": ent}
+        if defer:
+            pending = ent["used"]
+        else:
+            ent["buf"][:ent["used"]].zero_()
+    _tls.ustat = {"buf": ent["buf"], "off": 0, "unit": int(unit), "ent": ent, "pending": pending}
 
 
 def ustat_end():
@@ -298,6 +307,9 @@
     st = getattr(_tls, "ustat", None)
     if st is None or st.get("closed"):
         return None
+    if st.get("pending"):
+        st["buf"][:st["pending"]].zero_()
+        st["pending"] = 0
     unit = st["unit"]
     units = (nout + unit - 1) // unit
     nrep = USTAT_NREP
@@ -466,6 +478,8 @@
         p.depth_in, p.lddin = depth_in.data_ptr(), _ld(depth_in)
     p.y, p.ldy, p.out_f32 = out.data_ptr(), _ld(out), int(out_f32)
     p.epilogue = EPILOGUE
+    if not HEAD_TAIL and p.epilogue == 0 and B * Hout * Wout <= 8:
+        p.epilogue = 3
     p.io_f32 = int(f32)
     if f32:
         for t_, nm in ((x2, "x2"), (residual, "residual"), (depth_in, "depth_in")):
@@ -550,6 +564,9 @@
     return (out, stats) if rowstats else out
 
 
+HEAD_TAIL = os.environ.get("APTP_HEAD_TAIL", "1") != "0"
+
+
 def linear(x: torch.Tensor, pw: PackedWeight, **kw) -> torch.Tensor:
     B, L, C = x.shape
     out = kw.pop("out", None)
@@ -704,21 +721,39 @@
     return out
 
 
-def unet_prologue(sample: torch.Tensor, timesteps: torch.Tensor, freqs: torch.Tensor, cin_pad: int):
+IM2COL_K = 64
+
+
+def unet_prologue(sample: torch.Tensor, timesteps: torch.Tensor, freqs: torch.Tensor, cin_pad: int, *, im2col: bool = False,
+                  cast: Optional[torch.Tensor] = None):
     lib = _lib.load()
     assert sample.is_cuda and sample.dim() == 4 and sample.dtype in (torch.float32, torch.bfloat16)
     sample = sample.contiguous()
     B, C, H, W = sample.shape
-    t = timesteps.to(device=sample.device, dtype=torch.float32).contiguous()
+    p = UnetPrologueParams()
+    if HEAD_TAIL and timesteps.dtype == torch.int64 and timesteps.device == sample.device and timesteps.dim() == 1 \
+            and timesteps.shape[0] == B:
+        t = timesteps
+        p.timesteps_i64, p.timesteps_stride = 1, (t.stride(0) if B > 1 else 0)
+    else:
+        t = timesteps.to(device=sample.device, dtype=torch.float32).contiguous()
     assert t.numel() == B and freqs.dtype == torch.float32 and freqs.is_contiguous()
-    x = torch.empty(B, H, W, cin_pad, dtype=torch.bfloat16, device=sample.device)
+    x = torch.empty(B, H, W, IM2COL_K if im2col else cin_pad, dtype=torch.bfloat16, device=sample.device)
     temb = torch.empty(B, 2 * freqs.numel(), dtype=torch.bfloat16, device=sample.device)
-    p = UnetPrologueParams()
     p.sample, p.sample_bf16, p.x = sample.data_ptr(), int(sample.dtype == torch.bfloat16), x.data_ptr()
-    p.B, p.C, p.H, p.W, p.cin_pad = B, C, H, W, cin_pad
+    p.B, p.C, p.H, p.W, p.cin_pad, p.im2col = B, C, H, W, cin_pad, int(im2col)
     p.timesteps, p.freqs, p.half, p.t_emb = t.data_ptr(), freqs.data_ptr(), freqs.numel(), temb.data_ptr()
+    st = getattr(_tls, "ustat", None)
+    if st is not None and st.get("pending") and st["buf"].device == sample.device:
+        p.zero, p.zero_bytes = st["buf"].data_ptr(), 8 * round_up(st["pending"], 2)
+        st["pending"] = 0
+    cast_out = None
+    if cast is not None:
+        assert cast.is_cuda and cast.dtype == torch.float32 and cast.is_contiguous() and cast.numel() % 8 == 0 and cast.data_ptr() % 16 == 0
+        cast_out = torch.empty(cast.shape, dtype=torch.bfloat16, device=cast.device)
+        p.cast_src, p.cast_dst, p.cast_n = cast.data_ptr(), cast_out.data_ptr(), cast.numel()
     _lib.check(lib.aptp_unet_prologue(ctypes.byref(p), _stream()), "aptp_unet_prologue")
-    return x, temb
+    return (x, temb) if cast is None else (x, temb, cast_out)
 
 
 def unet_epilogue(y: torch.Tensor, channels: int, out_dtype: torch.dtype, out: Optional[torch.Tensor] = None) -> torch.Tensor:
@@ -805,10 +840,10 @@
 
 def pack_conv_in_im2col(w: torch.Tensor, bias: Optional[torch.Tensor], device=None) -> PackedWeight:
     O, C, KH, KW = w.shape
-    if (C, KH, KW) != (3, 3, 3):
-        raise ValueError(f"pack_conv_in_im2col: expected a [O, 3, 3, 3] weight, got {tuple(w.shape)}")
-    w2 = torch.zeros(O, 32, dtype=torch.float32, device=w.device)
-    w2[:, :27] = w.detach().float().permute(0, 2, 3, 1).reshape(O, 27)
+    if (KH, KW) != (3, 3) or C not in (3, 4):
+        raise ValueError(f"pack_conv_in_im2col: expected a [O, 3 or 4, 3, 3] weight, got {tuple(w.shape)}")
+    w2 = torch.zeros(O, 32 if C == 3 else IM2COL_K, dtype=torch.float32, device=w.device)
+    w2[:, :9 * C] = w.detach().float().permute(0, 2, 3, 1).reshape(O, 9 * C)
     return pack_weight(w2, None if bias is None else bias.detach(), device=device)
 
 
diff --git a/diffusion_pruning_amd/unet.py b/diffusion_pruning_amd/unet.py
--- a/diffusion_pruning_amd/unet.py
+++ b/diffusion_pruning_amd/unet.py
@@ -1294,6 +1294,8 @@
             cin_pad = ops.round_up(self.in_channels, 8)
             m = {"cin_pad": cin_pad}
             m["conv_in"] = ops.pack_weight(self.conv_in.weight.detach(), self.conv_in.bias.detach(), device=dev)
+            if self.in_channels == 4 and ops.ACT_DTYPE == torch.bfloat16:
+                m["conv_in_lin"] = ops.pack_conv_in_im2col(self.conv_in.weight.detach(), self.conv_in.bias.detach(), device=dev)
             te = self.time_embedding
             m["t1"] = ops.pack_weight(te.linear_1.weight.detach(), te.linear_1.bias.detach(), device=dev)
             m["t2"] = ops.pack_weight(te.linear_2.weight.detach(), te.linear_2.bias.detach(), device=dev)
@@ -1471,7 +1473,7 @@
                 for c in self.config["block_out_channels"]:
                     unit = math.gcd(unit, c // g) if c % g == 0 else 1
                 unit = self.__dict__["_ustat_unit"] = unit if unit >= 4 else 0
-            ops.ustat_begin(dev, unit)
+            ops.ustat_begin(dev, unit, defer=True)
         try:
             return self._forward_impl(sample, timestep, encoder_hidden_states, return_dict)
         finally:
@@ -1495,8 +1497,17 @@
         timesteps = timesteps.to(dev).expand(B)
         fused_io = sample.is_cuda and sample.dtype in (torch.float32, torch.bfloat16) and not torch.is_grad_enabled() \
             and ops.ACT_DTYPE == torch.bfloat16
+        conv_in_pw, ehs_cast = misc["conv_in"], None
         if fused_io:
-            x, t_emb = ops.unet_prologue(sample, timesteps, misc["freqs"], misc["cin_pad"])
+            im2col = ops.HEAD_TAIL and "conv_in_lin" in misc
+            ehs = encoder_hidden_states
+            if ops.HEAD_TAIL and torch.is_tensor(ehs) and ehs.dtype == torch.float32 and ehs.device == dev and ehs.is_contiguous() \
+                    and ehs.numel() % 8 == 0 and ehs.data_ptr() % 16 == 0:
+                x, t_emb, ehs_cast = ops.unet_prologue(sample, timesteps, misc["freqs"], misc["cin_pad"], im2col=im2col, cast=ehs)
+            else:
+                x, t_emb = ops.unet_prologue(sample, timesteps, misc["freqs"], misc["cin_pad"], im2col=im2col)
+            if im2col:
+                conv_in_pw = misc["conv_in_lin"]
         else:
             ang = timesteps.float()[:, None] * misc["freqs"][None, :]
             t_emb = torch.cat([torch.cos(ang), torch.sin(ang)], dim=-1).to(ops.ACT_DTYPE)
@@ -1513,13 +1524,13 @@
             ctx = encoder_hidden_states
         else:
             ehs_in = encoder_hidden_states.ehs if isinstance(encoder_hidden_states, CtxBundle) else encoder_hidden_states
-            ctx = self._project_context(ehs_in, bp, dev)
+            ctx = self._project_context(ehs_in if ehs_cast is None else ehs_cast, bp, dev)
 
         if x is None:
             x = torch.zeros(B, sample.shape[2], sample.shape[3], misc["cin_pad"], dtype=ops.ACT_DTYPE, device=dev)
             x[..., :self.in_channels] = sample.permute(0, 2, 3, 1)
         conv_in_dst = self._register_cat_slots(B, x.shape[1], x.shape[2], misc["conv_in"].N, dev)
-        h = _nchw(ops.conv_gemm(x, misc["conv_in"], out=conv_in_dst, colstats=True))
+        h = _nchw(ops.conv_gemm(x, conv_in_pw, out=conv_in_dst, colstats=True))
 
         down_block_res_samples = (h,)
         for blk in self.down_blocks:
diff --git a/include/aptp_hip.h b/include/aptp_hip.h
--- a/include/aptp_hip.h
+++ b/include/aptp_hip.h
@@ -165,6 +165,11 @@
   const float* freqs;
   int32_t half;
   void* t_emb;
+  int32_t timesteps_i64;
+  int64_t timesteps_stride;
+  void* zero; int64_t zero_bytes;
+  const float* cast_src; void* cast_dst; int64_t cast_n;
+  int32_t im2col;
 } AptpUnetPrologueParams;
 
 typedef struct {
@@ -175,6 +180,20 @@
 
 int aptp_unet_prologue(const AptpUnetPrologueParams* p, aptp_stream_t stream);
 int aptp_unet_epilogue(const AptpUnetEpilogueParams* p, aptp_stream_t stream);
+
+typedef struct {
+  const void* x; int64_t ldx;
+  const void* w; int64_t ldw;
+  const float* bias;
+  void* y; int64_t ldy;
+  int32_t M, N, K;
+  int32_t act;
+  int32_t out_f32;
+} AptpLinSkinnyParams;
+
+int aptp_lin_skinny(const AptpLinSkinnyParams* p, aptp_stream_t stream);
+int aptp_lin_skinny_supported(const AptpLinSkinnyParams* p);
+int aptp_conv_gemm_is_skinny(const AptpConvGemmParams* p);
 
 typedef struct {
   const void* q; int64_t q_stride_b, q_stride_l;
```

New measurement: 207.4 steps/s, median of 6. +1.0%, better.
